# YiwenShaoStephen/mergeNet

Hardware: AMD Instinct MI355X
Metric: merged Mpixels/sec at 1024x2048 (speculative fast path; proven path: value_proven_path) (higher is better)
Workload: dtype f32

## Files before the change

mergenet_amd/csrc/mergenet_hip.hip:

```cpp
#include <hip/hip_runtime.h>
#include <hip/hip_ext.h>

#include <math.h>
#include <stdio.h>
#include <stdlib.h>
#include <string.h>
#include <time.h>

#include "../../include/mergenet_hip.h"
#include "mn_device.h"
#include "mn_kernels_score.h"
#include "mn_kernels_merge.h"
#include "mn_kernels_finish.h"
#include "mn_kernels_output.h"
#include "mn_kernels_prepare.h"
#include "mn_kernels_instances.h"
#include "mn_kernels_cc.h"
#include "mn_kernels_tail.h"
#include "mn_kernels_exact.h"
#include "mn_kernels_reforder.h"

#define MN_NSCALARS 16
#define MN_STAT_BYTES ((((sizeof(Counters) + 15) & ~(size_t)15)) + MN_NSCALARS * sizeof(int) + 4 * sizeof(double))

#define MN_MAX_SUBROUNDS 64

static thread_local int g_last_status = MN_OK;

#define MN_HIP(expr)                                                                      \
  do {                                                                                    \
    hipError_t _e = (expr);                                                               \
    if (_e != hipSuccess) {                                                               \
      fprintf(stderr, "mergenet_hip: %s failed: %s (%s:%d)\n", #expr, hipGetErrorString(_e), \
              __FILE__, __LINE__);                                                        \
      g_last_status = MN_ERR_NO_DEVICE;                                                   \
      return MN_ERR_NO_DEVICE;                                                            \
    }                                                                                     \
  } while (0)

template <typename T>
struct HostBuf {
  T* p;
  explicit HostBuf(size_t n) : p(static_cast<T*>(calloc(n ? n : 1, sizeof(T)))) {}
  ~HostBuf() { free(p); }
  HostBuf(const HostBuf&) = delete;
  bool ok() const { return p != nullptr; }
  operator T*() const { return p; }
};

struct ImageCall {
  const void *d_class, *d_adj;
  int dtype;
  int class_dim, offset_dim, W, H, num_classes;
  int *d_mask, *d_objcls, *d_part;
  hipStream_t stream;
  bool has_offsets;
  int offs[2 * MN_MAX_OFFSETS];
  mn_options opts;
};

struct Queued { int mode, rounds, finish_limit, N; long long R0; bool speculate, want_cert; };

struct mn_context {
  int device;
  int maxH, maxW, maxC, maxO;
  size_t N, Rmax, cap;
  size_t cap_full;
  int gen_ready;
  size_t gen_bytes;
  size_t cc_cap;
  int debug_flags;
  size_t bytes;
  unsigned char *ocls, *cls0, *lpvalid, *matched, *pruned;
  int *osize, *parent, *mate, *root, *label, *mapbuf;
  float* lpsum;
  i64* lp_acc;
  u64 *ball, *bsub;
  RecList LA, LB;
  int* touched_list;
  int* fin_lists;
  int fin_lds_ready, tail_lds_ready;
  int* wire_counts;
  int core_radius;
  int ext_events;
  int cores_used;
  int cc_clean;
  HashTab T;
  int* block_count;
  double* partial;
  Counters* cnt;
  int* scalars;
  unsigned* gmax;
  unsigned* touch;
  unsigned* h_touch;
  float* theta;
  int* progress;
  u64* bg_key;
  double* lp_out;
  Counters* h_cnt;
  int* h_scalars;
  double* h_lp;
  size_t cc_sum_lds, oc_lds;
  unsigned char* statblk;
  unsigned char* h_statblk;
  int *cc_tcount, *cc_lcount;
  unsigned* cc_bits;
  int* cc_roots;
  int cc_sign_blocks;
  unsigned* cc_negbits;
  size_t cc_cap_max;
  hipEvent_t ev[12];
  struct Pending {
    int active;
    int rc;
    Queued queued;
    ImageCall call;
    mn_stats stats;
  } pend;
  hipEvent_t ev_done;
  struct Replay {
    int state;
    int capturing;
    unsigned char key[256];
    size_t key_bytes;
    hipGraph_t gA, gB;
    hipGraphExec_t eA, eB;
    hipStream_t cap;
    Queued queued;
  } replay;
  hipStream_t side;
  hipEvent_t ev_fork;
  ImgParams last_params;
  int last_valid;
  struct XWork {
    XState X;
    size_t n_pix, n_rec, n_cls_floats, hcap, arena_cap, leaf_cap;
    void* block;
    size_t bytes;
    XCtl* h_ctl;
    int lds_ready;
    int prerun;
    ImgParams* d_P;
    XState* d_X;
    int batch_cap;
    int arena_extra;
    int table_permille;
    int max_blocks;
  } xw;
  struct RWork {
    RoState S;
    void* block;
    size_t bytes;
    int n_pix; long long n_rec; int n_cls; long long arena_cap, heap_cap;
    int arena_per_pixel, heap_per_record;
    long long* h_ctl;
    RoState* d_S;
    int batch_cap;
  } rw;
  int tie_ref;
  int tie_used;
  float *d_class, *d_same;
  int *d_mask, *d_objcls, *d_part;
};

#define MN_DEFAULT_CORE_RADIUS 6

static double g_host_us[4];
static long long g_host_n[2];
static inline double host_now_us() {
  timespec ts;
  clock_gettime(CLOCK_MONOTONIC, &ts);
  return (double)ts.tv_sec * 1e6 + (double)ts.tv_nsec * 1e-3;
}

struct HostLaunchTimer {
  double t0;
  HostLaunchTimer() : t0(host_now_us()) {}
  ~HostLaunchTimer() { g_host_us[0] += host_now_us() - t0; g_host_n[0]++; }
};

static size_t next_pow2(size_t x) {
  size_t p = 1;
  while (p < x) p <<= 1;
  return p;
}

template <typename T>
static hipError_t dev_alloc(mn_context* c, T** p, size_t n) {
  const size_t b = (n * sizeof(T) + 255) & ~(size_t)255;
  c->bytes += b;
  return hipMalloc(reinterpret_cast<void**>(p), b);
}

static void x_free(mn_context* c) {
  XState& X = c->xw.X;
  if (c->xw.block) (void)hipFree(c->xw.block);
  if (X.mlog) (void)hipFree(X.mlog);
  if (c->xw.h_ctl) (void)hipHostFree(c->xw.h_ctl);
  c->bytes -= c->xw.bytes;
  const mn_context::XWork keep = c->xw;
  memset(&c->xw, 0, sizeof(c->xw));
  c->xw.d_P = keep.d_P; c->xw.d_X = keep.d_X; c->xw.batch_cap = keep.batch_cap;
  c->xw.arena_extra = keep.arena_extra; c->xw.table_permille = keep.table_permille; c->xw.max_blocks = keep.max_blocks;
}

static void r_free(mn_context* c) {
  if (c->rw.block) (void)hipFree(c->rw.block);
  if (c->rw.h_ctl) (void)hipHostFree(c->rw.h_ctl);
  c->bytes -= c->rw.bytes;
  const int ap = c->rw.arena_per_pixel, hp = c->rw.heap_per_record, bc = c->rw.batch_cap;
  RoState* ds = c->rw.d_S;
  memset(&c->rw, 0, sizeof(c->rw));
  c->rw.arena_per_pixel = ap; c->rw.heap_per_record = hp; c->rw.d_S = ds; c->rw.batch_cap = bc;
}

static int x_ensure(mn_context* c, int N, int O, int C) {
  mn_context::XWork& w = c->xw;
  const size_t NL = (size_t)N * O;
  if (NL >= 0xFFFFFFF0ull) return MN_ERR_CAPACITY;
  size_t B = 256;
  const size_t max_blocks = w.max_blocks > 0 ? (size_t)w.max_blocks : (size_t)MN_X_MAXBLOCKS;
  while ((NL + B - 1) / B > max_blocks) B <<= 1;
  const size_t NB = (NL + B - 1) / B;
  const size_t leaf_cap = NB * B + 1024;
  if (w.arena_extra <= 0) {
    w.arena_extra = 8 * O + 8;
    if (const char* e = getenv("MN_X_ARENA_EXTRA")) { const int v = atoi(e); if (v > 0) w.arena_extra = v; }
    w.table_permille = 600;
    if (const char* e = getenv("MN_X_TABLE_PERMILLE")) { const int v = atoi(e); if (v >= 50 && v <= 950) w.table_permille = v; }
  }
  const size_t nbuckets = (size_t)((double)NL * 1000.0 / (4.0 * (double)w.table_permille)) + 64;
  if (nbuckets * 4 >= 0xFFFFFFF0ull) return MN_ERR_CAPACITY;
  const size_t arena_cap = (size_t)N * (size_t)w.arena_extra + 65536;
  if (arena_cap >= 0xFFFFFFF0ull) return MN_ERR_CAPACITY;
  const size_t ovf_cap = NL / 256 + 4096;
  if (w.n_pix < (size_t)N || w.n_rec < NL || w.n_cls_floats < (size_t)N * C || w.hcap < nbuckets ||
      w.arena_cap < arena_cap || w.leaf_cap < leaf_cap) {
    x_free(c);
    XState& X = w.X;
    {
      const size_t al = ((size_t)N * O > (1u << 20)) ? ((size_t)2 << 20) : 4096;
      size_t off = 0;
      auto take = [&](size_t bytes) { const size_t o = off; off += (bytes + al - 1) / al * al; return o; };
      const size_t o_hs = take(nbuckets * 4 * sizeof(XSlot)), o_rec = take(NL * sizeof(XRec)),
                   o_arena = take(arena_cap * sizeof(unsigned)), o_leaf = take(leaf_cap * sizeof(unsigned)),
                   o_lp = take(((size_t)N * C + 64) * sizeof(float)), o_obj = take((size_t)N * sizeof(XObj)),
                   o_acap = take((size_t)N * sizeof(int)), o_ostamp = take((size_t)N * 2 * sizeof(unsigned)),
                   o_ovf = take(ovf_cap * sizeof(unsigned)), o_l1g = take((size_t)MN_X_MAXBLOCKS * sizeof(u64)),
                   o_tstack = take((size_t)MN_X_TSTACK * sizeof(u64)), o_free = take((size_t)MN_X_FREE_CLASSES * sizeof(unsigned)),
                   o_ctl = take(sizeof(XCtl));
      MN_HIP(hipMalloc(&w.block, off));
      w.bytes = off;
      c->bytes += off;
      char* b = static_cast<char*>(w.block);
      X.hs = reinterpret_cast<XSlot*>(b + o_hs); X.rec = reinterpret_cast<XRec*>(b + o_rec);
      X.arena = reinterpret_cast<unsigned*>(b + o_arena); X.leaf = reinterpret_cast<unsigned*>(b + o_leaf);
      X.lp = reinterpret_cast<float*>(b + o_lp); X.obj = reinterpret_cast<XObj*>(b + o_obj);
      X.acap = reinterpret_cast<int*>(b + o_acap); X.ostamp = reinterpret_cast<unsigned*>(b + o_ostamp);
      X.overflow = reinterpret_cast<unsigned*>(b + o_ovf); X.l1g = reinterpret_cast<u64*>(b + o_l1g);
      X.tstack = reinterpret_cast<u64*>(b + o_tstack); X.ctl = reinterpret_cast<XCtl*>(b + o_ctl);
      X.freeheads = reinterpret_cast<unsigned*>(b + o_free);
    }
    MN_HIP(hipHostMalloc(reinterpret_cast<void**>(&w.h_ctl), sizeof(XCtl)));
    w.n_pix = N; w.n_rec = NL; w.n_cls_floats = (size_t)N * C; w.hcap = nbuckets; w.arena_cap = arena_cap;
    w.leaf_cap = leaf_cap;
    X.overflow_cap = (int)ovf_cap;
  }
  XState& X = w.X;
  X.nb = (unsigned)nbuckets;
  X.arena_cap = arena_cap;
  X.Blog = 0;
  while (((size_t)1 << X.Blog) < B) X.Blog++;
  X.NB = (int)NB;
  X.NBpad = (int)((NB + 63) / 64 * 64);
  X.NG = X.NBpad / 64;
  X.NL = (unsigned)NL;
  X.parent = c->parent;
  X.dbg = getenv("MN_X_FORCE_RELOCATE") ? 1 : 0;
  if (getenv("MN_X_MERGELOG") && !X.mlog) {
    if (hipMalloc(reinterpret_cast<void**>(&X.mlog), (size_t)N * 16) == hipSuccess) X.mlog_cap = N;
    else X.mlog = nullptr;
// ... 291 lines not shown
}

static int begin_call(mn_context* c, const ImageCall& call, bool entry_ok, mn_stats* stats, ImgParams* P) {
  int rc = check_args(c, call);
  if (rc == MN_OK && (!call.d_class || !call.d_adj || !dtype_ok(call.dtype, true) || !entry_ok)) rc = MN_ERR_ARGUMENT;
  if (stats) { memset(stats, 0, sizeof(*stats)); stats->status = rc; stats->total_logprob = NAN; }
  if (rc != MN_OK) { g_last_status = rc; return rc; }
  MN_HIP(hipSetDevice(c->device));
  fill_params(P, call);
  return MN_OK;
}

static long long count_records(const ImageCall& call) {
  long long r = 0;
  for (int k = 0; k < call.offset_dim; k++) {
    const long long hh = call.H - abs(call.offs[2 * k]), ww = call.W - abs(call.offs[2 * k + 1]);
    if (hh > 0 && ww > 0) r += hh * ww;
  }
  return r;
}

static inline unsigned grid_for(size_t n, unsigned block) { return (unsigned)((n + block - 1) / block); }

struct FillList {
  FillJobs j;
  size_t largest = 0;
  FillList() { j.count = 0; }
  void add(void* p, size_t bytes, unsigned char byte) {
    if (!bytes) return;
    j.ptr[j.count] = p;
    j.bytes[j.count] = bytes;
    j.pattern[j.count] = 0x01010101u * byte;
    j.count++;
    if (bytes > largest) largest = bytes;
  }
  bool full() const { return j.count == MN_FILL_JOBS; }
  void launch(hipStream_t st) {
    if (!j.count) return;
    unsigned blocks = grid_for(largest / 16 + 1, 256 * 4);
    if (blocks > 4096) blocks = 4096;
    if (blocks < 1) blocks = 1;
    hipLaunchKernelGGL(mn_fill_many, dim3(blocks), dim3(256), 0, st, j);
    j.count = 0;
    largest = 0;
  }
};

static ObjState obj_state(mn_context* c) {
  ObjState S;
  S.ocls = c->ocls; S.osize = c->osize; S.parent = c->parent; S.lpsum = c->lpsum;
  S.lpvalid = c->lpvalid;
  return S;
}

template <bool FIRST>
static void launch_edge_pass(mn_context* c, const ImgParams& P, hipStream_t st, u64* out, int s) {
  const int* progress = c->progress;
  const dim3 g(grid_for(P.N, 256)), b(256);
  const dim3 gx(8 * ((grid_for(P.N, 256) + 7) / 8));
  const unsigned char* cls0 = c->ocls;
  const unsigned char* matched = c->matched;
  const bool fast = P.omf > 0.0f && P.sdb == 0.0f && !(c->debug_flags & 1);
  if (fast && P.O == 10 && !P.clip)
    hipLaunchKernelGGL((mn_edge_pass_fast<10, FIRST, false>), gx, b, 0, st, P, cls0, matched, out,
                       progress, s);
  else if (fast && P.O == 10)
    hipLaunchKernelGGL((mn_edge_pass_fast<10, FIRST, true>), gx, b, 0, st, P, cls0, matched, out,
                       progress, s);
  else if (fast && P.O == 16 && !P.clip)
    hipLaunchKernelGGL((mn_edge_pass_fast<16, FIRST, false>), gx, b, 0, st, P, cls0, matched, out,
                       progress, s);
  else if (fast && P.O == 16)
    hipLaunchKernelGGL((mn_edge_pass_fast<16, FIRST, true>), gx, b, 0, st, P, cls0, matched, out,
                       progress, s);
  else
    hipLaunchKernelGGL(mn_edge_pass_generic<FIRST>, g, b, 0, st, P, obj_state(c), matched, out, progress, s);
}

static int run_phase_a(mn_context* c, const ImgParams& P, hipStream_t st, bool edge,
                       FillList* fills = nullptr, bool components = false) {
  const int N = P.N;
  FillList own;
  if (!fills) fills = &own;
  if (!components) {
    fills->add(c->lpvalid, N, 0);
    fills->add(c->matched, N, 0);
  }
  fills->launch(st);
  if (components) {
    if (!c->ext_events) MN_HIP(hipEventRecord(c->ev[0], st));
    return MN_OK;
  }
  hipLaunchKernelGGL(mn_init_objects, dim3(grid_for(N, 256)), dim3(256), 0, st, N, c->osize,
                     c->parent, c->mate);
  MN_HIP(hipEventRecord(c->ev[0], st));
  {
    const unsigned blocks = grid_for((size_t)(N >> 2) > 0 ? (size_t)(N >> 2) : 1, 256);
    hipLaunchKernelGGL(mn_class_pass, dim3(blocks), dim3(256), 0, st, P, c->ocls);
  }
  MN_HIP(hipEventRecord(c->ev[1], st));
  if (edge) {
    launch_edge_pass<true>(c, P, st, c->ball, 0);
  }
  MN_HIP(hipEventRecord(c->ev[2], st));
  MN_HIP(hipMemcpyAsync(c->cls0, c->ocls, N, hipMemcpyDeviceToDevice, st));
  MN_HIP(hipGetLastError());
  return MN_OK;
}

static int read_counters(mn_context* c, hipStream_t st) {
  MN_HIP(hipMemcpyAsync(c->h_cnt, c->cnt, sizeof(Counters), hipMemcpyDeviceToHost, st));
  MN_HIP(hipStreamSynchronize(st));
  return MN_OK;
}

static int build_list(mn_context* c, const ImgParams& P, hipStream_t st, size_t cap, RecList L,
                      const RecList* src, int Rsrc, int* Rout) {
  ObjState S = obj_state(c);
  HashTab T = c->T;
  T.mask = (unsigned)(cap - 1);
  FillList f;
  f.add(T.key, cap * sizeof(u64), 0xFF);
  f.add(T.S, cap * sizeof(i64), 0);
  f.add(T.touched, cap, 0);
  f.add(&c->cnt->n_records, sizeof(int), 0);
  f.add(c->ball, (size_t)P.N * sizeof(u64), 0);
  f.add(c->gmax, 64 * sizeof(unsigned), 0);
  f.launch(st);
  if (!src)
    hipLaunchKernelGGL(mn_build_from_pixels, dim3(grid_for(P.N, 256)), dim3(256), 0, st, P, S, T);
  else
    hipLaunchKernelGGL(mn_rebuild, dim3(grid_for(Rsrc, MN_REBUILD_ITEMS)), dim3(256), 0, st, S, *src,
                       Rsrc, (const unsigned char*)c->matched, T, L, c->ball, c->gmax, c->cnt,  0);
  if (cap <= (1u << 16))
    hipLaunchKernelGGL(mn_compact<1>, dim3(grid_for(cap, 256)), dim3(256), 0, st, P, S, T, L,
                       c->ball, c->gmax, c->cnt, (const int*)nullptr, (int*)nullptr);
  else
    hipLaunchKernelGGL(mn_compact<4>, dim3(grid_for(cap, MN_COMPACT_SLOTS)), dim3(256), 0, st, P, S, T, L,
                       c->ball, c->gmax, c->cnt, (const int*)nullptr, (int*)nullptr);
  MN_HIP(hipGetLastError());
  if (read_counters(c, st) != MN_OK) return MN_ERR_NO_DEVICE;
  *Rout = c->h_cnt->n_records;
  return MN_OK;
}

static size_t gsum_stride(int N) {
#ifdef MN_GSUM_SKEW
  return ((((size_t)N / 4 + 63) / 64) | 1) * 64;
#else
  return (size_t)N;
#endif
}

template <int PX, int DT, bool LG = false>
static void launch_sign(mn_context* c, const ImgParams& P, hipStream_t st, bool cls, bool lean_cls) {
  const int N = P.N, ngroups = (N + PX - 1) / PX;
  const dim3 g(grid_for(ngroups, MN_CC_SIGN_THREADS)), b(MN_CC_SIGN_THREADS);
  ClsOut CO;
  CO.ocls = lean_cls ? nullptr : c->ocls; CO.cls0 = c->cls0; CO.lpvalid = lean_cls ? nullptr : c->lpvalid;
  CO.gsum = reinterpret_cast<int*>(c->lpsum);
  CO.gstride = gsum_stride(P.N);
  const bool plain = (DT != MN_DTYPE_F32 || LG || !P.clip) && P.sdb == 0.0f;
#define MN_LAUNCH_SIGN(PLAINV, CLSV)                                                                    \
  do {                                                                                                \
    if (c->ext_events)                                                                                \
      hipExtLaunchKernelGGL((mn_cc_sign<PX, PLAINV, (CLSV) && PX >= 4, DT, LG>), g, b, 0, st, c->ev[0], c->ev[10], 0, \
                            P, c->cc_bits, c->cc_negbits, c->scalars + 6, c->partial, CO); \
    else                                                                                              \
      hipLaunchKernelGGL((mn_cc_sign<PX, PLAINV, (CLSV) && PX >= 4, DT, LG>), g, b, 0, st, P, c->cc_bits, c->cc_negbits, \
                         c->scalars + 6, c->partial, CO);                                             \
  } while (0)
  if (plain && cls) MN_LAUNCH_SIGN(true, true);
  else if (plain) MN_LAUNCH_SIGN(true, false);
  else if (cls) MN_LAUNCH_SIGN(false, true);
  else MN_LAUNCH_SIGN(false, false);
#undef MN_LAUNCH_SIGN
}

static int sweep_px(const mn_context* c, const ImgParams& P) {
  if (!((P.N & 3) == 0 && P.W >= 4)) return 1;
  if (P.dtype != MN_DTYPE_F32 && !(c->debug_flags & 256) && (P.N & 7) == 0 && (P.W & 7) == 0 &&
      ((reinterpret_cast<uintptr_t>(P.cls) | reinterpret_cast<uintptr_t>(P.same)) & 15) == 0)
    return 8;
  return 4;
}

template <bool LG>
static void launch_sweep_lg(mn_context* c, const ImgParams& P, hipStream_t st, int px, bool cls, bool lean_cls) {
#define MN_SWEEP_DT(PXV)                                                                         \
  do {                                                                                           \
    if (P.dtype == MN_DTYPE_F16) launch_sign<PXV, MN_DTYPE_F16, LG>(c, P, st, cls, lean_cls);    \
    else launch_sign<PXV, MN_DTYPE_BF16, LG>(c, P, st, cls, lean_cls);                           \
  } while (0)
  if (P.dtype == MN_DTYPE_F32) {
    if (px == 4) launch_sign<4, MN_DTYPE_F32, LG>(c, P, st, cls, lean_cls);
    else launch_sign<1, MN_DTYPE_F32, LG>(c, P, st, false, false);
  } else if (px == 8) MN_SWEEP_DT(8);
  else if (px == 4) MN_SWEEP_DT(4);
  else { cls = false; lean_cls = false; MN_SWEEP_DT(1); }
#undef MN_SWEEP_DT
}
static void launch_sweep(mn_context* c, const ImgParams& P, hipStream_t st, int px, bool cls, bool lean_cls) {
  if (P.logits) launch_sweep_lg<true>(c, P, st, px, cls, lean_cls);
  else launch_sweep_lg<false>(c, P, st, px, cls, lean_cls);
}

template <int PX>
static void launch_cc_hook(mn_context* c, const ImgParams& P, hipStream_t st, unsigned kmask,
                           const unsigned* hook_bits = nullptr, hipEvent_t hook_done = nullptr) {
  const int N = P.N, ngroups = (N + PX - 1) / PX;
  const dim3 gx(8 * ((grid_for(ngroups, 256) + 7) / 8));
  if (hook_done)
    hipExtLaunchKernelGGL(mn_cc_hook<PX>, gx, dim3(256), 0, st, nullptr, hook_done, 0, P,
                          hook_bits ? hook_bits : (const unsigned*)c->cc_bits, c->parent, kmask);
  else
    hipLaunchKernelGGL(mn_cc_hook<PX>, gx, dim3(256), 0, st, P, hook_bits ? hook_bits : (const unsigned*)c->cc_bits,
                       c->parent, kmask);
}

enum CcUse {
  CC_WAITED,
  CC_QUEUED_COMPACT,
  CC_QUEUED_TAIL,
  CC_CORES
};

static int run_components(mn_context* c, const ImgParams& P, hipStream_t& st, CcUse use) {
  const bool wait = use == CC_WAITED, with_ball = use == CC_WAITED;
  const bool with_compact = use == CC_WAITED || use == CC_QUEUED_COMPACT;
  const bool fork_before_sums = use == CC_QUEUED_TAIL, cores = use == CC_CORES;
  const int N = P.N;
  ObjState S = obj_state(c);
  const dim3 b(256);
  const bool four = P.W % 4 == 0;
  int kh = -1, kv = -1, dv = 0;
  for (int k = 0; k < P.O; k++) {
    if (kh < 0 && P.di[k] == 0 && P.dj[k] == 1) kh = k;
    if (kv < 0 && P.dj[k] == 0 && (P.di[k] == 1 || P.di[k] == -1)) { kv = k; dv = P.di[k]; }
  }
  const bool few_events = (c->debug_flags & 2) != 0;
  const bool lean = (c->debug_flags & 16) != 0;
  const dim3 tiles((P.W + 63) / 64, (P.H + MN_CC_TILE_ROWS - 1) / MN_CC_TILE_ROWS);
  const int px = sweep_px(c, P);
  const bool sweep4 = px >= 4;
  const size_t sign_blocks = grid_for((size_t)(N / px), MN_CC_SIGN_THREADS);
  c->cc_sign_blocks = (int)(sign_blocks * (MN_CC_SIGN_THREADS / 64));
  int* clsmin = c->root;
  int* clsmax = c->mapbuf;
  const bool fused_cls = sweep4;
  const bool lean_cls = fused_cls && !cores;
  launch_sweep(c, P, st, px, fused_cls, lean_cls);
  if (!few_events && !c->ext_events) MN_HIP(hipEventRecord(c->ev[10], st));
  const unsigned* lbits = c->cc_bits;
  unsigned kshort = 0u;
  if (cores) {
    if (!fused_cls) {
      const unsigned blocks = grid_for((size_t)(N >> 2) > 0 ? (size_t)(N >> 2) : 1, 256);
      hipLaunchKernelGGL(mn_class_pass, dim3(blocks), dim3(256), 0, st, P, c->cls0);
    }
    unsigned* bits2 = reinterpret_cast<unsigned*>(c->label);
    for (int k = 0; k < P.O; k++)
      if (c->core_radius < 0 || (abs(P.di[k]) <= c->core_radius && abs(P.dj[k]) <= c->core_radius)) kshort |= 1u << k;
    hipLaunchKernelGGL(mn_core_clean, dim3(grid_for(N, 256)), b, 0, st, P, (const unsigned*)c->cc_bits,
                       (const unsigned char*)c->cls0, c->pruned, kshort);
    hipLaunchKernelGGL(mn_core_bits, dim3(grid_for(N, 256)), b, 0, st, P, (const unsigned char*)c->pruned,
                       (const unsigned*)c->cc_bits, (const unsigned char*)c->cls0, bits2);
    lbits = bits2;
  }
  hipStream_t real = st;
  if (c->replay.capturing) {
    MN_HIP(hipStreamBeginCapture(c->replay.cap, hipStreamCaptureModeThreadLocal));
    st = c->replay.cap;
  }
  unsigned kmask = P.O >= 32 ? 0xFFFFFFFFu : ((1u << P.O) - 1u);
  const bool fork_ext = fork_before_sums && c->ext_events && !c->replay.capturing;
  bool fork_by_hook = false;
  hipLaunchKernelGGL(mn_cc_tiles, tiles, dim3(MN_CC_TILE_ROWS * 64), 0, st, P, lbits, c->parent, kh, kv, dv,
                     c->osize, c->lp_acc, clsmin, clsmax, c->matched);
  if (kh >= 0 || kv >= 0) {
    hipLaunchKernelGGL(mn_cc_borders, tiles, dim3(128), 0, st, P, lbits, c->parent, kh, kv, dv);
    if (kh >= 0) kmask &= ~(1u << kh);
    if (kv >= 0) kmask &= ~(1u << kv);
  }
  hipLaunchKernelGGL(mn_cc_flatten, dim3(grid_for((size_t)(N >> 2) > 0 ? (size_t)(N >> 2) : 1, 256)), b, 0, st, N, c->parent);
  fork_by_hook = fork_ext && kmask;
  if (kmask) {
    if (four) launch_cc_hook<4>(c, P, st, kmask, lbits, fork_by_hook ? c->ev_fork : nullptr);
    else launch_cc_hook<1>(c, P, st, kmask, lbits, fork_by_hook ? c->ev_fork : nullptr);
  }
  if (c->replay.capturing) {
    MN_HIP(hipStreamEndCapture(c->replay.cap, &c->replay.gA));
    MN_HIP(hipGraphInstantiate(&c->replay.eA, c->replay.gA, nullptr, nullptr, 0));
    MN_HIP(hipGraphLaunch(c->replay.eA, real));
    st = real;
  }
  HashTab T = c->T;
  T.mask = (unsigned)(c->cc_cap - 1);
  if (!few_events && !lean) MN_HIP(hipEventRecord(c->ev[7], st));
  if (fork_before_sums) {
    if (!fork_by_hook) MN_HIP(hipEventRecord(c->ev_fork, st));
    MN_HIP(hipStreamWaitEvent(c->side, c->ev_fork, 0));
    st = c->side;
    if (c->replay.capturing) {
      MN_HIP(hipStreamBeginCapture(c->replay.cap, hipStreamCaptureModeThreadLocal));
      st = c->replay.cap;
    }
  }
  if (!few_events && !lean) MN_HIP(hipEventRecord(c->ev[11], st));
  {
    const size_t lds = (size_t)MN_CC_SUM_SLOTS * (P.C + 1) * sizeof(u64);
    if (lds > c->cc_sum_lds) {
      MN_HIP(hipFuncSetAttribute(reinterpret_cast<const void*>(mn_cc_class_sums),
                                 hipFuncAttributeMaxDynamicSharedMemorySize, (int)lds));
      MN_HIP(hipFuncSetAttribute(reinterpret_cast<const void*>(mn_cc_sums),
                                 hipFuncAttributeMaxDynamicSharedMemorySize, (int)lds));
      c->cc_sum_lds = lds;
    }
    const unsigned blocks = grid_for((size_t)(N >> 2) > 0 ? (size_t)(N >> 2) : 1, MN_CC_SUM_THREADS);
    if (fused_cls)
      hipLaunchKernelGGL(mn_cc_sums, dim3((blocks + MN_CC_SUMS_ITERS - 1) / MN_CC_SUMS_ITERS), dim3(MN_CC_SUM_THREADS), lds, st, P, S,
                         (const unsigned char*)c->cls0, (const int*)reinterpret_cast<int*>(c->lpsum), gsum_stride(P.N),
                         c->lp_acc, clsmin, clsmax, cores ? (const unsigned char*)c->pruned : (const unsigned char*)nullptr);
    else
      hipLaunchKernelGGL(mn_cc_class_sums, dim3(blocks), dim3(MN_CC_SUM_THREADS), lds, st, P, S, c->cls0,
                         c->lp_acc, clsmin, clsmax);
  }
  if (!few_events && !lean) MN_HIP(hipEventRecord(c->ev[8], st));
  if (!cores)
  {
    if (sweep4)
      hipLaunchKernelGGL(mn_cc_cross<4>, dim3((unsigned)grid_for((size_t)N / 4, MN_CC_CROSS_THREADS)), dim3(MN_CC_CROSS_THREADS),
                         0, st, P, (const int*)c->parent, T, (const unsigned*)c->cc_negbits, c->scalars + 6, c->cc_tcount);
    else
      hipLaunchKernelGGL(mn_cc_cross<1>, dim3((unsigned)grid_for((size_t)N, MN_CC_CROSS_THREADS)), dim3(MN_CC_CROSS_THREADS),
                         0, st, P, (const int*)c->parent, T, (const unsigned*)c->cc_negbits, c->scalars + 6, c->cc_tcount);
  }
  if (!few_events && !lean) MN_HIP(hipEventRecord(c->ev[9], st));
  hipLaunchKernelGGL(mn_cc_finish, dim3(grid_for((size_t)(N >> 4) > 0 ? (size_t)(N >> 4) : 1, 256)), b, 0, st, P, S,
                     (const unsigned char*)c->matched, (const i64*)c->lp_acc,
                     (const int*)clsmin, (const int*)clsmax, c->mate, cores ? (int*)nullptr : c->cc_roots,
                     c->scalars + 8, c->scalars + 6, lean_cls ? (const unsigned char*)c->cls0 : (const unsigned char*)nullptr);
  if (cores) {
    const unsigned all = P.O >= 32 ? 0xFFFFFFFFu : ((1u << P.O) - 1u);
    if (kshort != all) {
      MN_HIP(hipMemsetAsync(c->matched, 0, (size_t)N, st));
      hipLaunchKernelGGL(mn_core_check, dim3(grid_for(N, 256)), b, 0, st, P, (const int*)c->parent, lbits, c->matched);
      hipLaunchKernelGGL(mn_core_dissolve, dim3(grid_for(N, 256)), b, 0, st, P, S,
                         (const unsigned char*)c->matched, c->scalars + 9);
    }
    hipLaunchKernelGGL(mn_count_cross_edges, dim3(grid_for(N, 256)), b, 0, st, P, (const int*)c->parent, c->touch);
  }
  if (with_compact)
    hipLaunchKernelGGL(mn_compact<4>, dim3(grid_for(c->cc_cap, MN_COMPACT_SLOTS)), dim3(256), 0, st, P, S,
                       T, c->LA, with_ball ? c->ball : (u64*)nullptr, c->gmax, c->cnt,
                       (const int*)c->cc_tcount, c->cc_lcount);
  MN_HIP(hipGetLastError());
  if (!wait) return 0;
  MN_HIP(hipMemcpyAsync(c->h_scalars, c->scalars, MN_NSCALARS * sizeof(int), hipMemcpyDeviceToHost, st));
  MN_HIP(hipMemcpyAsync(c->h_cnt, c->cnt, sizeof(Counters), hipMemcpyDeviceToHost, st));
  MN_HIP(hipStreamSynchronize(st));
  if (c->h_scalars[6] != 0 || c->h_scalars[7] != 0) {
    MN_HIP(hipMemsetAsync(c->cnt, 0, sizeof(Counters), st));
    return 1;
  }
  return 0;
}

static int exact_setup(mn_context* c, const ImgParams& P, hipStream_t st) {
  int rc = x_ensure(c, P.N, P.O, P.C);
  if (rc != MN_OK) return rc;
  mn_context::XWork& w = c->xw;
  XState& X = w.X;
  const size_t N = (size_t)P.N;
  MN_HIP(hipMemsetAsync(X.hs, 0xFF, (size_t)X.nb * 4 * sizeof(XSlot), st));
  MN_HIP(hipMemsetAsync(X.leaf, 0, (((size_t)X.NB << X.Blog) + 1024) * sizeof(unsigned), st));
  MN_HIP(hipMemsetAsync(X.ostamp, 0, (size_t)N * 2 * sizeof(unsigned), st));
  MN_HIP(hipMemsetAsync(X.freeheads, 0xFF, MN_X_FREE_CLASSES * sizeof(unsigned), st));
  memset(w.h_ctl, 0, sizeof(XCtl));
  w.h_ctl->ttrack = getenv("MN_X_NO_TIE_TRACKING") ? 0 : 1;
  w.h_ctl->bump = 0ull;
  MN_HIP(hipMemcpyAsync(X.ctl, w.h_ctl, sizeof(XCtl), hipMemcpyHostToDevice, st));
  hipLaunchKernelGGL(mn_x_init_objects, dim3(grid_for(N, 256)), dim3(256), 0, st, P, X, c->cls0);
  MN_HIP(hipEventRecord(c->ev[1], st));
  hipLaunchKernelGGL(mn_x_init_records, dim3(grid_for((size_t)X.NL, 256)), dim3(256), 0, st, P, X);
  MN_HIP(hipEventRecord(c->ev[2], st));
  MN_HIP(hipGetLastError());
  return MN_OK;
}

static int exact_loop(mn_context** cs, int n, const ImgParams* Ps, hipStream_t st, unsigned char* full) {
  mn_context::XWork& w0 = cs[0]->xw;
  if (w0.batch_cap < n) {
    if (w0.d_P) (void)hipFree(w0.d_P);
    if (w0.d_X) (void)hipFree(w0.d_X);
    w0.d_P = nullptr; w0.d_X = nullptr;
    MN_HIP(hipMalloc(reinterpret_cast<void**>(&w0.d_P), (size_t)n * sizeof(ImgParams)));
    MN_HIP(hipMalloc(reinterpret_cast<void**>(&w0.d_X), (size_t)n * sizeof(XState)));
    w0.batch_cap = n;
  }
  size_t lds = 0;
  long long max_total = 0;
  {
    HostBuf<XState> hx((size_t)n);
    if (!hx.ok()) return MN_ERR_INTERNAL;
    for (int i = 0; i < n; i++) {
      const XState& X = cs[i]->xw.X;
      hx[i] = X;
      const size_t l = MN_X_LDS_BYTES(X.NBpad);
      if (l > lds) lds = l;
      const long long mt = 8LL * (long long)X.NL + 65536;
      if (mt > max_total) max_total = mt;
    }
    hipError_t e1 = hipMemcpyAsync(w0.d_P, Ps, (size_t)n * sizeof(ImgParams), hipMemcpyHostToDevice, st);
    hipError_t e2 = hipMemcpyAsync(w0.d_X, hx, (size_t)n * sizeof(XState), hipMemcpyHostToDevice, st);
    hipError_t e3 = hipStreamSynchronize(st);
    MN_HIP(e1); MN_HIP(e2); MN_HIP(e3);
  }
  if (!w0.lds_ready) {
    MN_HIP(hipFuncSetAttribute(reinterpret_cast<const void*>(mn_x_run),
                               hipFuncAttributeMaxDynamicSharedMemorySize, 160 * 1024));
    w0.lds_ready = 1;
  }
  long long per_launch = 1LL << 24;
  if (const char* e = getenv("MN_X_BUDGET")) { const long long v = atoll(e); if (v > 0) per_launch = v; }
  const long long max_launches = 1 << 20;
  for (long long it = 0; it < max_launches; it++) {
    long long most = 0;
    bool any = false;
    for (int i = 0; i < n; i++) {
      mn_context::XWork& w = cs[i]->xw;
      if (it > 0 && w.h_ctl->status != MN_X_BUDGET) continue;
      any = true;
      if (w.h_ctl->steps > most) most = w.h_ctl->steps;
      hipLaunchKernelGGL(mn_x_build_l1, dim3(w.X.NB), dim3(64), 0, st, w.X);
    }
    if (!any) break;
    const long long left = max_total - most;
    if (left <= 0) {
      fprintf(stderr, "mergenet_hip: exact engine exceeded %lld steps\n", max_total);
      return MN_ERR_INTERNAL;
    }
    const long long budget = left < per_launch ? left : per_launch;
    hipLaunchKernelGGL(mn_x_run, dim3((unsigned)n), dim3(64), lds, st, (const ImgParams*)w0.d_P, (const XState*)w0.d_X, budget);
    MN_HIP(hipGetLastError());
    for (int i = 0; i < n; i++)
      MN_HIP(hipMemcpyAsync(cs[i]->xw.h_ctl, cs[i]->xw.X.ctl, sizeof(XCtl), hipMemcpyDeviceToHost, st));
    MN_HIP(hipStreamSynchronize(st));
    bool all_done = true;
    for (int i = 0; i < n; i++) {
      const int status = cs[i]->xw.h_ctl->status;
      if (status == MN_X_DONE) continue;
      all_done = false;
      if (status == MN_X_BUDGET) continue;
      if (status == MN_X_ARENA_FULL || status == MN_X_HASH_FULL) {
        if (getenv("MN_TRACE_EXACT"))
          fprintf(stderr, "exact engine: out of %s after %lld steps (image %d of the batch): workspace grows, run repeated\n",
                  status == MN_X_ARENA_FULL ? "adjacency arena" : "pair table", cs[i]->xw.h_ctl->steps, i);
        full[i] = (unsigned char)status;
        continue;
      }
      fprintf(stderr, "mergenet_hip: exact engine stopped with status %d after %lld steps\n", status, cs[i]->xw.h_ctl->steps);
      return MN_ERR_INTERNAL;
    }
    if (all_done) break;
  }
  for (int i = 0; i < n; i++)
    if (cs[i]->xw.h_ctl->status != MN_X_DONE && !full[i]) return MN_ERR_INTERNAL;
  return MN_OK;
}

static int exact_run(mn_context** cs, int n, const ImgParams* Ps, hipStream_t st) {
  HostBuf<mn_context*> sub((size_t)n); HostBuf<ImgParams> subP((size_t)n); HostBuf<unsigned char> full((size_t)n);
  int rc = (sub.ok() && subP.ok() && full.ok()) ? MN_OK : MN_ERR_INTERNAL, m = n;
  for (int i = 0; i < n && rc == MN_OK; i++) { sub[i] = cs[i]; subP[i] = Ps[i]; }
  for (int attempt = 0; rc == MN_OK && m > 0; attempt++) {
    if (attempt == 8) { rc = MN_ERR_CAPACITY; break; }
    for (int i = 0; i < m && rc == MN_OK; i++) rc = exact_setup(sub[i], subP[i], st);
    if (rc != MN_OK) break;
    memset(full, 0, (size_t)m);
    rc = exact_loop(sub, m, subP, st, full);
    if (rc != MN_OK) break;
    int k = 0;
    for (int i = 0; i < m; i++) {
      if (!full[i]) continue;
      mn_context::XWork& w = sub[i]->xw;
      if (full[i] == MN_X_ARENA_FULL) w.arena_extra *= 2;
      else if (w.table_permille > 100) w.table_permille = w.table_permille * 2 / 3;
      else { rc = MN_ERR_CAPACITY; break; }
// ... 561 lines not shown
                       A.cur, c->cc_lcount, c->label, c->fin_lists, c->cnt, max_steps, c->scalars, pl.finish_limit,
                       (const unsigned char*)c->cls0, (const int*)c->mate, (const int*)c->cc_roots, nbe,
                       (const double*)c->partial, c->lp_out, pl.want_cert ? 1 : 0, c->label, call.d_objcls);
  } else {
    if (A.mode != MN_MODE_EXACT && A.R > 0 && !call.opts.no_handover_refresh &&
        !(A.mode == MN_MODE_COMPONENTS && A.rounds == 0))
      hipLaunchKernelGGL(mn_rec_refresh, dim3(grid_for(A.R, 256)), dim3(256), 0, A.st, P, S, A.cur, A.R);
    if (A.R <= MN_FIN2_MAXR) {
      if (!c->fin_lds_ready) {
        MN_HIP(hipFuncSetAttribute(reinterpret_cast<const void*>(mn_finisher_lds),
                                   hipFuncAttributeMaxDynamicSharedMemorySize, MN_FIN2_MAXR * 12));
        c->fin_lds_ready = 1;
      }
      hipLaunchKernelGGL(mn_finisher_lds, dim3(1), dim3(MN_FIN2_THREADS), MN_FIN2_MAXR * 12, A.st, P, S, A.cur, A.R, c->label,
                         c->fin_lists, c->cnt, max_steps, pl.speculate ? (const int*)&c->cnt->n_records : (const int*)nullptr,
                         (const int*)(c->scalars + 6), pl.finish_limit,
                         (A.mode == MN_MODE_COMPONENTS && A.rounds == 0) ? c->cc_lcount : (int*)nullptr);
    } else {
      if (A.mode == MN_MODE_COMPONENTS || A.cores)
        MN_HIP(hipMemsetAsync(c->mapbuf, 0xFF, (size_t)P.N * sizeof(int), A.st));
      hipLaunchKernelGGL(mn_finisher, dim3(1), dim3(MN_FIN_THREADS), 0, A.st, P, S, A.cur, A.R, c->mapbuf,
                         c->touched_list, c->cnt, max_steps);
    }
  }
  if (!pl.lean) MN_HIP(hipEventRecord(c->ev[3], A.st));
  return MN_OK;
}

static int launch_output(mn_context* c, const ImgParams& P, const Plan& pl, const Attempt& A, const ImageCall& call) {
  const int N = P.N;
  const ObjState S = obj_state(c);
  const unsigned char* pruned = NULL;
  if (call.opts.variant == MN_VARIANT_PYSEGMENTER) {
    MN_HIP(hipMemsetAsync(c->bg_key, 0, sizeof(u64), A.st));
    hipLaunchKernelGGL(mn_prune_find_background, dim3(grid_for(N, 256)), dim3(256), 0, A.st, P, S, c->bg_key);
    hipLaunchKernelGGL(mn_prune_mark, dim3(grid_for(N, 256)), dim3(256), 0, A.st, P, S,
                       call.opts.prune_threshold, (const u64*)c->bg_key, c->pruned, c->cnt);
    pruned = c->pruned;
  }
  if (!pl.fused_tail) {
    const int nblk = (int)grid_for(N, MN_SCAN_ITEMS);
    hipLaunchKernelGGL(mn_rank_count, dim3(nblk), dim3(256), 0, A.st, N, S, pruned, c->block_count, c->scalars + 2);
    hipLaunchKernelGGL(mn_rank_scan, dim3(1), dim3(1024), 0, A.st, nblk, c->block_count, c->scalars + 1);
    hipLaunchKernelGGL(mn_rank_assign, dim3(nblk), dim3(256), 0, A.st, N, S, pruned,
                       (const int*)c->block_count, c->label, call.d_objcls);
  }
  {
    const bool need_root = pl.want_cert && !pl.fused_tail && !A.cc_certificate();
    int* root_out = need_root ? c->root : nullptr;
    const bool aligned = (N & 3) == 0 && ((reinterpret_cast<uintptr_t>(call.d_mask) | reinterpret_cast<uintptr_t>(call.d_objcls) |
                                           reinterpret_cast<uintptr_t>(call.d_part)) & 15) == 0;
    if (aligned)
      hipLaunchKernelGGL(mn_write_mask4, dim3(grid_for((size_t)N / 4, 256)), dim3(256), 0, A.st, N, (const int*)c->parent,
                         (const int*)c->label, (const int*)(c->scalars + 1), root_out, call.d_mask, call.d_part, call.d_objcls);
    else
      hipLaunchKernelGGL(mn_write_mask, dim3(grid_for(N, 256)), dim3(256), 0, A.st, N, (const int*)c->parent,
                         (const int*)c->label, (const int*)(c->scalars + 1), root_out, call.d_mask, call.d_part, call.d_objcls);
  }
  return MN_OK;
}

static int launch_certificate(mn_context* c, const ImgParams& P, const Plan& pl, const Attempt& A) {
  const int N = P.N, R = A.R;
  const ObjState S = obj_state(c);
  if (!pl.want_cert || pl.fused_tail) {
  } else if (A.cc_certificate()) {
    const int nbe = c->cc_sign_blocks;
    hipLaunchKernelGGL(mn_cc_certificate, dim3(1), dim3(MN_CC_CERT_THREADS), 0, A.st, P, S, (const unsigned char*)c->cls0,
                       (const int*)c->mate, (const int*)c->cc_roots, (const int*)(c->scalars + 8), nbe,
                       (const double*)c->partial, (const Counters*)c->cnt, c->lp_out, c->scalars);
  } else {
    const bool four = P.W % 4 == 0;
    const int vb = (int)grid_for(four ? (size_t)N / 4 : (size_t)N, four ? MN_VERIFY4_THREADS : 256);
    if (four)
      hipLaunchKernelGGL(mn_verify_edges4, dim3(vb), dim3(MN_VERIFY4_THREADS), 0, A.st, P, S,
                         (const unsigned char*)c->cls0, (const int*)c->root, c->partial, c->scalars);
    else
      hipLaunchKernelGGL(mn_verify_edges, dim3(vb), dim3(256), 0, A.st, P, S,
                         (const unsigned char*)c->cls0, (const int*)c->root, c->partial, c->scalars);
    hipLaunchKernelGGL(mn_verify_reduce, dim3(1), dim3(256), 0, A.st, vb, (const double*)c->partial, P.omf, c->lp_out);
    if (pl.xengine)
      hipLaunchKernelGGL(mn_x_verify_records, dim3(grid_for((size_t)c->xw.X.NL, 256)), dim3(256), 0, A.st, P,
                         c->xw.X, c->scalars);
  }
  if (pl.want_cert && !pl.fused_tail && R > 0)
    hipLaunchKernelGGL(mn_verify_records, dim3(grid_for(R, 256)), dim3(256), 0, A.st, P, S, A.cur, R,
                       c->scalars, pl.speculate ? (const int*)&c->cnt->n_records : (const int*)nullptr);
  if (!pl.lean) MN_HIP(hipEventRecord(c->ev[4], A.st));
  MN_HIP(hipGetLastError());
  return MN_OK;
}

static int close_attempt(mn_context* c, const ImageCall& call, const Plan& pl, Attempt& A, mn_stats* stats, bool defer) {
  hipStream_t st = A.st;
  const Queued q = {A.mode, A.rounds, pl.finish_limit, call.W * call.H, pl.R0, pl.speculate, pl.want_cert};
  MN_HIP(hipMemcpyAsync(c->h_statblk, c->statblk, MN_STAT_BYTES, hipMemcpyDeviceToHost, st));
  if (pl.fused_tail) {
    A.post.launch(st);
    c->cc_clean = 1;
  }
  if (c->replay.capturing) {
    MN_HIP(hipStreamEndCapture(c->replay.cap, &c->replay.gB));
    MN_HIP(hipGraphInstantiate(&c->replay.eB, c->replay.gB, nullptr, nullptr, 0));
    MN_HIP(hipGraphLaunch(c->replay.eB, c->side));
    st = c->side;
    c->replay.capturing = 0;
    c->replay.state = 2;
    c->replay.queued = q;
  }
  if (defer && pl.speculate) {
    MN_HIP(hipEventRecord(c->ev_done, st));
    c->pend.queued = q;
    return MN_PENDING;
  }
  MN_HIP(hipStreamSynchronize(st));
  return segment_read_back(c, &call.opts, q, stats);
}

static int segment_attempt(mn_context* c, const ImageCall& call, mn_stats* stats, int force_mode, bool speculate, bool defer = false) {
  ImgParams P;
  int rc = begin_call(c, call, call.d_mask && call.d_objcls, stats, &P);
  if (rc != MN_OK) return rc;
  static const int env_flags = getenv("MN_DEBUG_FLAGS_OR") ? atoi(getenv("MN_DEBUG_FLAGS_OR")) : 0;
  c->debug_flags = call.opts.debug_flags | env_flags;
  c->ext_events = !(call.opts.debug_flags & 2) && !(call.opts.debug_flags & 128);
  c->core_radius = call.opts.core_radius != 0 ? call.opts.core_radius : MN_DEFAULT_CORE_RADIUS;
  const Plan pl = make_plan(call, force_mode, speculate);
  c->tie_ref = pl.xengine ? call.opts.tie_order : MN_TIES_LOWEST_ID;
  c->tie_used = 0; c->cores_used = 0;
  if (!pl.xengine && (rc = ensure_fast(c)) != MN_OK) return rc;
  if (!pl.speculate && !pl.xengine && (rc = ensure_general(c)) != MN_OK) return rc;
  Attempt A = {call.stream, pl.mode, pl.mode == MN_MODE_ROUNDS && pl.cores_ok, c->LA, c->LB, 0, 0};
  build_clear_list(c, P, pl, A);
  if ((rc = run_first_phase(c, P, pl, A)) != MN_OK) return rc;
  if ((rc = run_round0(c, P, pl, A)) != MN_OK) return rc;
  if ((rc = run_rounds(c, P, pl, A)) != MN_OK) return rc;
  if ((rc = launch_finisher(c, P, pl, A, call)) != MN_OK) return rc;
  if ((rc = launch_output(c, P, pl, A, call)) != MN_OK) return rc;
  if ((rc = launch_certificate(c, P, pl, A)) != MN_OK) return rc;
  c->last_params = P; c->last_valid = 1;
  return close_attempt(c, call, pl, A, stats, defer);
}

static int replay_launch(mn_context* c, const ImageCall& call) {
  ImgParams P;
  const int rc = begin_call(c, call, true, nullptr, &P);
  if (rc != MN_OK) return rc;
  const hipStream_t st = call.stream;
  c->debug_flags = call.opts.debug_flags;
  c->ext_events = !(call.opts.debug_flags & 2) && !(call.opts.debug_flags & 128);
  c->cores_used = 0;
  const bool timed = !(call.opts.debug_flags & 2) && !c->ext_events;
  if (timed) MN_HIP(hipEventRecord(c->ev[0], st));
  launch_sweep(c, P, st, sweep_px(c, P), true, true);
  if (timed) MN_HIP(hipEventRecord(c->ev[10], st));
  MN_HIP(hipGraphLaunch(c->replay.eA, st));
  MN_HIP(hipEventRecord(c->ev_fork, st));
  MN_HIP(hipStreamWaitEvent(c->side, c->ev_fork, 0));
  MN_HIP(hipGraphLaunch(c->replay.eB, c->side));
  MN_HIP(hipEventRecord(c->ev_done, c->side));
  c->last_params = P; c->last_valid = 1;
  c->pend.queued = c->replay.queued;
  memset(&c->pend.stats, 0, sizeof(c->pend.stats));
  c->pend.active = 1;
  return MN_OK;
}

extern "C" int mn_segment_launch_t(mn_context* c, const void* d_class_pred, int class_dim,
                                   const void* d_adj_pred, int offset_dim, int dtype, int W, int H,
                                   int num_classes, const int* offset_list, int* d_mask,
                                   int* d_object_class, int* d_partition, const mn_options* opts,
                                   void* stream) {
  if (!c || c->pend.active || !dtype_ok(dtype, true)) { g_last_status = MN_ERR_ARGUMENT; return MN_ERR_ARGUMENT; }
  HostLaunchTimer host_timer;
  mn_context::Pending& q = c->pend;
  q.call = ImageCall{d_class_pred, d_adj_pred, dtype, class_dim, offset_dim, W, H, num_classes, d_mask, d_object_class, d_partition};
  image_call(&q.call, offset_list, opts, stream);
  const mn_options& o = q.call.opts;
  mn_context::Replay& rp = c->replay;
  const bool want_replay = (o.debug_flags & 32) && (o.debug_flags & 16) && offset_list &&
                           offset_dim > 0 && offset_dim <= MN_MAX_OFFSETS && W % 4 == 0;
  unsigned char key[256];
  size_t kb = 0;
  if (want_replay) {
    memset(key, 0, sizeof(key));
    const void* ptrs[6] = {d_class_pred, d_adj_pred, d_mask, d_object_class, d_partition, stream};
    const int dims[6] = {class_dim, offset_dim, W, H, num_classes, dtype};
    memcpy(key + kb, ptrs, sizeof(ptrs)); kb += sizeof(ptrs);
    memcpy(key + kb, dims, sizeof(dims)); kb += sizeof(dims);
    memcpy(key + kb, &o, sizeof(o)); kb += sizeof(o);
    const size_t ob = sizeof(int) * 2 * (size_t)offset_dim;
    if (kb + ob <= sizeof(key)) { memcpy(key + kb, q.call.offs, ob); kb += ob; } else kb = 0;
  }
  const bool same_key = want_replay && kb && rp.state >= 1 && rp.key_bytes == kb && memcmp(rp.key, key, kb) == 0;
  if (same_key && rp.state == 2 && c->cc_clean) return replay_launch(c, q.call);
  if (want_replay && kb && !same_key) drop_replay_graphs(rp);
  rp.capturing = (same_key && rp.state == 1 && c->cc_clean) ? 1 : 0;
  const int was_clean = c->cc_clean;
  const int rc = segment_attempt(c, q.call, &q.stats, 0, true, true);
  if (rp.capturing) {
    hipGraph_t open_graph = nullptr;
    if (hipStreamEndCapture(rp.cap, &open_graph) == hipSuccess && open_graph) (void)hipGraphDestroy(open_graph);
    (void)hipGetLastError();
    rp.capturing = 0;
    rp.state = 0;
  }
  if (want_replay && kb && rp.state == 0 && rc == MN_PENDING && was_clean && c->cc_clean &&
      o.variant == MN_VARIANT_CSEGMENT && (W * H) % 4 == 0) {
    memcpy(rp.key, key, kb);
    rp.key_bytes = kb;
    rp.state = 1;
  }
  if (rc == MN_PENDING) { q.active = 1; return MN_OK; }
  if (rc < 0 && rc != MN_ERR_NO_BACKGROUND) return rc;
  q.active = 2;
  q.rc = rc;
  return MN_OK;
}

extern "C" int mn_segment_launch(mn_context* c, const float* d_class_pred, int class_dim,
                                 const float* d_adj_pred, int offset_dim, int W, int H,
                                 int num_classes, const int* offset_list, int* d_mask,
                                 int* d_object_class, int* d_partition, const mn_options* opts,
                                 void* stream) {
  return mn_segment_launch_t(c, d_class_pred, class_dim, d_adj_pred, offset_dim, MN_DTYPE_F32, W, H, num_classes,
                             offset_list, d_mask, d_object_class, d_partition, opts, stream);
}

extern "C" int mn_segment_finish(mn_context* c, mn_stats* stats) {
  if (!c || !c->pend.active) { g_last_status = MN_ERR_ARGUMENT; return MN_ERR_ARGUMENT; }
  const double t_in = host_now_us();
  double t_synced = t_in;
  mn_context::Pending& q = c->pend;
  const mn_options& o = q.call.opts;
  int rc;
  const bool explicit_mode = o.mode == MN_MODE_EXACT || o.mode == MN_MODE_ROUNDS || o.mode == MN_MODE_COMPONENTS;
  const bool must_prove = o.require_proof > 0 || (o.require_proof == 0 && !explicit_mode);
  if (q.active == 2) {
    rc = q.rc;
  } else {
    MN_HIP(hipSetDevice(c->device));
    MN_HIP(hipEventSynchronize(c->ev_done));
    t_synced = host_now_us();
    memset(&q.stats, 0, sizeof(q.stats));
    rc = segment_read_back(c, &o, q.queued, &q.stats);
    if (rc == MN_RETRY_ROUNDS && must_prove)
      rc = segment_attempt(c, q.call, &q.stats, MN_MODE_EXACT, false);
    else if (rc == MN_RETRY_ROUNDS || rc == MN_RETRY_WAIT)
      rc = segment_attempt(c, q.call, &q.stats, rc == MN_RETRY_ROUNDS ? MN_MODE_ROUNDS : 0, false);
  }
  if (rc == MN_OK && must_prove && q.stats.proof == 0) {
    rc = segment_attempt(c, q.call, &q.stats, MN_MODE_EXACT, false);
    if (rc == MN_ERR_CAPACITY) rc = MN_ERR_UNPROVEN;
    if (rc == MN_ERR_UNPROVEN) { q.stats.status = rc; g_last_status = rc; }
  }
  if (rc == MN_OK && o.require_proof > 0 && q.stats.proof == MN_PROOF_SEQUENTIAL_TIES) {
    if (o.variant == MN_VARIANT_CSEGMENT) {
      ImageCall again = q.call;
      again.opts.tie_order = MN_TIES_REFERENCE;
      rc = segment_attempt(c, again, &q.stats, MN_MODE_EXACT, false);
      if (rc == MN_ERR_CAPACITY) rc = MN_ERR_UNPROVEN;
    } else {
      rc = MN_ERR_UNPROVEN;
    }
    if (rc == MN_ERR_UNPROVEN) { q.stats.status = rc; g_last_status = rc; }
  }
  if (stats) *stats = q.stats;
  q.active = 0;
  g_host_us[1] += t_synced - t_in; g_host_us[2] += host_now_us() - t_synced; g_host_n[1]++;
  return rc;
}

extern "C" int mn_segment_device_t(mn_context* c, const void* d_class_pred, int class_dim,
                                   const void* d_adj_pred, int offset_dim, int dtype, int W, int H,
                                   int num_classes, const int* offset_list, int* d_mask,
                                   int* d_object_class, int* d_partition, const mn_options* opts,
                                   void* stream, mn_stats* stats) {
  int rc = MN_ERR_ARGUMENT;
  if (!c || !c->pend.active)
    rc = mn_segment_launch_t(c, d_class_pred, class_dim, d_adj_pred, offset_dim, dtype, W, H, num_classes,
                             offset_list, d_mask, d_object_class, d_partition, opts, stream);
  if (rc != MN_OK) {
    if (stats) { memset(stats, 0, sizeof(*stats)); stats->status = rc; stats->total_logprob = NAN; }
    return rc;
  }
  return mn_segment_finish(c, stats);
}

extern "C" int mn_segment_device(mn_context* c, const float* d_class_pred, int class_dim,
                                 const float* d_adj_pred, int offset_dim, int W, int H,
                                 int num_classes, const int* offset_list, int* d_mask,
                                 int* d_object_class, int* d_partition, const mn_options* opts,
                                 void* stream, mn_stats* stats) {
  return mn_segment_device_t(c, d_class_pred, class_dim, d_adj_pred, offset_dim, MN_DTYPE_F32, W, H, num_classes,
                             offset_list, d_mask, d_object_class, d_partition, opts, stream, stats);
}

extern "C" int mn_segment_exact_batch_t(mn_context** ctxs, int count, const void* const* d_class_pred, int class_dim,
                                        const void* const* d_adj_pred, int offset_dim, int dtype, int W, int H,
                                        int num_classes, const int* offset_list, int* const* d_mask,
                                        int* const* d_object_class, int* const* d_partition, const mn_options* opts,
                                        void* stream, mn_stats* stats) {
  ImageCall shared = {nullptr, nullptr, dtype, class_dim, offset_dim, W, H, num_classes};
  image_call(&shared, offset_list, opts, stream);
  shared.opts.mode = MN_MODE_EXACT;
  const mn_options& o = shared.opts;
  if (!ctxs || count <= 0 || count > 4096 || !d_class_pred || !d_adj_pred || !d_mask || !d_object_class ||
// ... 58 lines not shown
    int n2 = 0;
    for (int i = 0; i < count; i++) {
      if (out[i].status != MN_OK || out[i].proof != MN_PROOF_SEQUENTIAL_TIES) continue;
      if (!ref_possible) {
        out[i].status = MN_ERR_UNPROVEN;
        if (rc == MN_OK) rc = MN_ERR_UNPROVEN;
        continue;
      }
      rc_ctx[n2] = ctxs[i]; rc_P[n2] = Ps[i]; rc_idx[n2] = i; n2++;
    }
    const int r2 = n2 > 0 ? redo_in_reference_order(rc_ctx, n2, rc_P, st, true) : MN_OK;
    if (r2 == MN_ERR_CAPACITY) {
      for (int j = 0; j < n2; j++) out[rc_idx[j]].status = MN_ERR_UNPROVEN;
      if (rc == MN_OK) rc = MN_ERR_UNPROVEN;
    } else if (r2 != MN_OK) {
      g_last_status = r2;
      return r2;
    }
    for (int j = 0; j < n2 && r2 == MN_OK; j++) {
      const int i = rc_idx[j];
      ctxs[i]->xw.prerun = 2;
      const int r = segment_attempt(ctxs[i], calls[i], &out[i], MN_MODE_EXACT, false);
      ctxs[i]->xw.prerun = 0;
      if (r != MN_OK && rc == MN_OK) rc = r;
    }
  }
  g_last_status = rc;
  return rc;
}

extern "C" int mn_segment_exact_batch(mn_context** ctxs, int count, const float* const* d_class_pred, int class_dim,
                                      const float* const* d_adj_pred, int offset_dim, int W, int H, int num_classes,
                                      const int* offset_list, int* const* d_mask, int* const* d_object_class,
                                      int* const* d_partition, const mn_options* opts, void* stream,
                                      mn_stats* stats) {
  return mn_segment_exact_batch_t(ctxs, count, reinterpret_cast<const void* const*>(d_class_pred), class_dim,
                                  reinterpret_cast<const void* const*>(d_adj_pred), offset_dim, MN_DTYPE_F32, W, H,
                                  num_classes, offset_list, d_mask, d_object_class, d_partition, opts, stream, stats);
}

extern "C" int mn_score_device_t(mn_context* c, const void* d_class_pred, int class_dim,
                                 const void* d_adj_pred, int offset_dim, int dtype, int W, int H,
                                 int num_classes, const int* offset_list, const mn_options* opts,
                                 void* stream, unsigned char* d_cls_out,
                                 unsigned long long* d_best_out, float* ms_class_pass,
                                 float* ms_edge_pass) {
  ImageCall call = {d_class_pred, d_adj_pred, dtype, class_dim, offset_dim, W, H, num_classes};
  image_call(&call, offset_list, opts, stream);
  ImgParams P;
  int rc = begin_call(c, call, true, nullptr, &P);
  if (rc != MN_OK) return rc;
  const hipStream_t st = call.stream;
  c->debug_flags = call.opts.debug_flags;
  if ((rc = ensure_fast(c)) != MN_OK || (rc = run_phase_a(c, P, st, true)) != MN_OK) return rc;
  if (d_cls_out) MN_HIP(hipMemcpyAsync(d_cls_out, c->ocls, P.N, hipMemcpyDeviceToDevice, st));
  if (d_best_out)
    MN_HIP(hipMemcpyAsync(d_best_out, c->ball, (size_t)P.N * sizeof(u64), hipMemcpyDeviceToDevice, st));
  MN_HIP(hipStreamSynchronize(st));
  float ms = 0;
  (void)hipEventElapsedTime(&ms, c->ev[0], c->ev[1]);
  if (ms_class_pass) *ms_class_pass = ms;
  (void)hipEventElapsedTime(&ms, c->ev[1], c->ev[2]);
  if (ms_edge_pass) *ms_edge_pass = ms;
  g_last_status = MN_OK;
  return MN_OK;
}

extern "C" int mn_score_device(mn_context* c, const float* d_class_pred, int class_dim,
                               const float* d_adj_pred, int offset_dim, int W, int H,
                               int num_classes, const int* offset_list, const mn_options* opts,
                               void* stream, unsigned char* d_cls_out,
                               unsigned long long* d_best_out, float* ms_class_pass,
                               float* ms_edge_pass) {
  return mn_score_device_t(c, d_class_pred, class_dim, d_adj_pred, offset_dim, MN_DTYPE_F32, W, H, num_classes,
                           offset_list, opts, stream, d_cls_out, d_best_out, ms_class_pass, ms_edge_pass);
}

extern "C" int mn_sweep_device_t(mn_context* c, const void* d_class_pred, int class_dim,
                                 const void* d_adj_pred, int offset_dim, int dtype, int W, int H, int num_classes,
                                 const int* offset_list, const mn_options* opts, void* stream,
                                 unsigned* d_bits_out, float* d_neg_out, unsigned char* d_cls_out,
                                 int* d_gsum_out, double* logsum_out, int* info_out) {
  ImageCall call = {d_class_pred, d_adj_pred, dtype, class_dim, offset_dim, W, H, num_classes};
  image_call(&call, offset_list, opts, stream);
  ImgParams P;
  const int rc = begin_call(c, call, d_bits_out && d_neg_out, nullptr, &P);
  if (rc != MN_OK) return rc;
  hipStream_t st = static_cast<hipStream_t>(stream);
  const int N = P.N;
  if (ensure_fast(c) != MN_OK) return MN_ERR_NO_DEVICE;
  c->debug_flags = call.opts.debug_flags | 2;
  c->ext_events = 0;
  c->cc_clean = 0;
  const int px = sweep_px(c, P);
  const bool four = px >= 4;
  const bool fused_cls = four;
  const size_t sign_blocks = grid_for((size_t)(N / px), MN_CC_SIGN_THREADS);
  const size_t sign_waves = sign_blocks * (MN_CC_SIGN_THREADS / 64);
  MN_HIP(hipMemsetAsync(c->scalars, 0, MN_NSCALARS * sizeof(int), st));
  launch_sweep(c, P, st, px, fused_cls, false);
  MN_HIP(hipMemsetD32Async(reinterpret_cast<hipDeviceptr_t>(d_neg_out), 0x7FC00000, (size_t)P.O * N, st));
  hipLaunchKernelGGL(mn_cc_export_neg, dim3((unsigned)grid_for((size_t)N, 256)), dim3(256), 0, st, P,
                     (const unsigned*)c->cc_negbits, d_neg_out);
  MN_HIP(hipMemcpyAsync(d_bits_out, c->cc_bits, (size_t)N * sizeof(unsigned), hipMemcpyDeviceToDevice, st));
  if (d_cls_out && fused_cls) MN_HIP(hipMemcpyAsync(d_cls_out, c->cls0, (size_t)N, hipMemcpyDeviceToDevice, st));
  if (d_gsum_out && fused_cls)
    MN_HIP(hipMemcpy2DAsync(d_gsum_out, (size_t)(N / 4) * sizeof(int), c->lpsum, gsum_stride(N) * sizeof(int),
                            (size_t)(N / 4) * sizeof(int), (size_t)P.C, hipMemcpyDeviceToDevice, st));
  HostBuf<double> hp(sign_waves * 2);
  if (!hp.ok()) return MN_ERR_INTERNAL;
  MN_HIP(hipMemcpyAsync(hp, c->partial, sign_waves * 2 * sizeof(double), hipMemcpyDeviceToHost, st));
  MN_HIP(hipMemcpyAsync(c->h_scalars, c->scalars, MN_NSCALARS * sizeof(int), hipMemcpyDeviceToHost, st));
  MN_HIP(hipStreamSynchronize(st));
  double t = 0.0;
  for (size_t b = 0; b < sign_waves; b++) t += hp[2 * b];
  if (logsum_out) *logsum_out = t;
  if (info_out) { info_out[0] = px; info_out[1] = fused_cls ? 1 : 0; info_out[2] = c->h_scalars[6]; }
  MN_HIP(hipGetLastError());
  g_last_status = MN_OK;
  return MN_OK;
}

extern "C" int mn_sweep_device(mn_context* c, const float* d_class_pred, int class_dim,
                               const float* d_adj_pred, int offset_dim, int W, int H, int num_classes,
                               const int* offset_list, const mn_options* opts, void* stream,
                               unsigned* d_bits_out, float* d_neg_out, unsigned char* d_cls_out,
                               int* d_gsum_out, double* logsum_out, int* info_out) {
  return mn_sweep_device_t(c, d_class_pred, class_dim, d_adj_pred, offset_dim, MN_DTYPE_F32, W, H, num_classes,
                           offset_list, opts, stream, d_bits_out, d_neg_out, d_cls_out, d_gsum_out, logsum_out, info_out);
}

extern "C" int mn_sweep_time_device_t(mn_context* c, const void* const* d_class_pred, const void* const* d_adj_pred,
                                      int dtype, int n_inputs, int class_dim, int offset_dim, int W, int H,
                                      int num_classes, const int* offset_list, const mn_options* opts, void* stream,
                                      int reps, float* us_per_launch) {
  const bool ok = d_class_pred && d_adj_pred && n_inputs >= 1 && reps >= 1 && us_per_launch;
  ImageCall call = {ok ? d_class_pred[0] : nullptr, ok ? d_adj_pred[0] : nullptr, dtype, class_dim, offset_dim, W, H, num_classes};
  image_call(&call, offset_list, opts, stream);
  ImgParams P;
  const int rc = begin_call(c, call, ok, nullptr, &P);
  if (rc != MN_OK) return rc;
  hipStream_t st = static_cast<hipStream_t>(stream);
  if (ensure_fast(c) != MN_OK) return MN_ERR_NO_DEVICE;
  c->debug_flags = call.opts.debug_flags | 2;
  c->ext_events = 0;
  c->cc_clean = 0;
  MN_HIP(hipMemsetAsync(c->scalars, 0, MN_NSCALARS * sizeof(int), st));
  for (int phase = 0; phase < 2; phase++) {
    const int n = phase == 0 ? (reps + 9) / 10 : reps;
    if (phase == 1) MN_HIP(hipEventRecord(c->ev[0], st));
    for (int i = 0; i < n; i++) {
      call.d_class = d_class_pred[i % n_inputs]; call.d_adj = d_adj_pred[i % n_inputs];
      fill_params(&P, call);
      launch_sweep(c, P, st, sweep_px(c, P), true, true);
    }
    if (phase == 1) MN_HIP(hipEventRecord(c->ev[1], st));
  }
  MN_HIP(hipStreamSynchronize(st));
  float ms = 0;
  MN_HIP(hipEventElapsedTime(&ms, c->ev[0], c->ev[1]));
  *us_per_launch = ms * 1e3f / (float)reps;
  MN_HIP(hipGetLastError());
  g_last_status = MN_OK;
  return MN_OK;
}

extern "C" int mn_sweep_time_device(mn_context* c, const float* const* d_class_pred, const float* const* d_adj_pred,
                                    int n_inputs, int class_dim, int offset_dim, int W, int H, int num_classes,
                                    const int* offset_list, const mn_options* opts, void* stream, int reps,
                                    float* us_per_launch) {
  return mn_sweep_time_device_t(c, reinterpret_cast<const void* const*>(d_class_pred),
                                reinterpret_cast<const void* const*>(d_adj_pred), MN_DTYPE_F32, n_inputs, class_dim,
                                offset_dim, W, H, num_classes, offset_list, opts, stream, reps, us_per_launch);
}

extern "C" int mn_exact_phase_a_device_t(mn_context* c, const void* d_class_pred, int class_dim,
                                         const void* d_adj_pred, int offset_dim, int dtype, int W, int H,
                                         int num_classes, const int* offset_list, const mn_options* opts,
                                         void* stream, unsigned char* d_cls_out, float* d_oml_out,
                                         float* d_prio_out) {
  ImageCall call = {d_class_pred, d_adj_pred, dtype, class_dim, offset_dim, W, H, num_classes};
  image_call(&call, offset_list, opts, stream);
  ImgParams P;
  int rc = begin_call(c, call, d_oml_out && d_prio_out, nullptr, &P);
  if (rc != MN_OK) return rc;
  hipStream_t st = static_cast<hipStream_t>(stream);
  if ((rc = exact_setup(c, P, st)) != MN_OK) { g_last_status = rc; return rc; }
  hipLaunchKernelGGL(mn_x_export_phase_a, dim3(grid_for((size_t)P.N * P.O, 256)), dim3(256), 0, st, P, c->xw.X,
                     d_oml_out, d_prio_out, d_cls_out);
  MN_HIP(hipGetLastError());
  MN_HIP(hipStreamSynchronize(st));
  g_last_status = MN_OK;
  return MN_OK;
}

extern "C" int mn_exact_phase_a_device(mn_context* c, const float* d_class_pred, int class_dim,
                                       const float* d_adj_pred, int offset_dim, int W, int H,
                                       int num_classes, const int* offset_list, const mn_options* opts,
                                       void* stream, unsigned char* d_cls_out, float* d_oml_out,
                                       float* d_prio_out) {
  return mn_exact_phase_a_device_t(c, d_class_pred, class_dim, d_adj_pred, offset_dim, MN_DTYPE_F32, W, H, num_classes,
                                   offset_list, opts, stream, d_cls_out, d_oml_out, d_prio_out);
}

static int ensure_staging(mn_context* c) {
  if (c->d_class) return MN_OK;
  MN_HIP(dev_alloc(c, &c->d_class, c->N * (size_t)c->maxC));
  MN_HIP(dev_alloc(c, &c->d_same, c->N * (size_t)c->maxO));
  MN_HIP(dev_alloc(c, &c->d_mask, c->N));
  MN_HIP(dev_alloc(c, &c->d_objcls, c->N));
  MN_HIP(dev_alloc(c, &c->d_part, c->N));
  return MN_OK;
}

extern "C" int mn_segment_host(mn_context* c, const float* class_pred, int class_dim,
                               const float* adj_pred, int offset_dim, int W, int H, int num_classes,
                               const int* offset_list, int* mask, int* object_class, int* partition,
                               const mn_options* opts, mn_stats* stats) {
  ImageCall call = {class_pred, adj_pred, MN_DTYPE_F32, class_dim, offset_dim, W, H, num_classes};
  image_call(&call, offset_list, opts, NULL);
  opts = &call.opts;
  int rc = check_args(c, call);
  if (rc == MN_OK && (!class_pred || !adj_pred || !mask || !object_class)) rc = MN_ERR_ARGUMENT;
  if (rc != MN_OK) { g_last_status = rc; if (stats) { memset(stats, 0, sizeof(*stats)); stats->status = rc; } return rc; }
  MN_HIP(hipSetDevice(c->device));
  rc = ensure_staging(c);
  if (rc != MN_OK) return rc;
  const size_t N = (size_t)W * H;
  MN_HIP(hipMemcpy(c->d_class, class_pred, N * num_classes * sizeof(float), hipMemcpyHostToDevice));
  MN_HIP(hipMemcpy(c->d_same, adj_pred, N * offset_dim * sizeof(float), hipMemcpyHostToDevice));
  rc = mn_segment_device(c, c->d_class, num_classes, c->d_same, offset_dim, W, H, num_classes,
                         offset_list, c->d_mask, c->d_objcls, c->d_part, opts, NULL, stats);
  if (rc != MN_OK && rc != MN_ERR_NO_BACKGROUND && rc != MN_ERR_UNPROVEN) return rc;
  MN_HIP(hipMemcpy(mask, c->d_mask, N * sizeof(int), hipMemcpyDeviceToHost));
  MN_HIP(hipMemcpy(object_class, c->d_objcls, N * sizeof(int), hipMemcpyDeviceToHost));
  if (partition) MN_HIP(hipMemcpy(partition, c->d_part, N * sizeof(int), hipMemcpyDeviceToHost));
  return rc;
}

extern "C" void c_run_segmentation(float* class_pred, int class_dim, float* adj_pred, int offset_dim,
                                   int img_width, int img_height, int num_classes, int* offset_list,
                                   int* output, int* object_class, float same_different_bias,
                                   float object_merge_factor, float merge_logprob_bias) {
  struct Cached { mn_context* c = NULL; ~Cached() { if (c) mn_destroy(c); } };
  static thread_local Cached holder;
  mn_context*& cached = holder.c;
  if (img_width <= 0 || img_height <= 0 || num_classes <= 0 || offset_dim <= 0) {
    g_last_status = MN_ERR_ARGUMENT;
    fprintf(stderr, "c_run_segmentation: %s\n", mn_status_string(MN_ERR_ARGUMENT));
    return;
  }
  if (cached && ((size_t)img_width * img_height > cached->N || num_classes > cached->maxC ||
                 offset_dim > cached->maxO)) {
    mn_destroy(cached);
    cached = NULL;
  }
  if (!cached) {
    int dev = 0;
    (void)hipGetDevice(&dev);
    cached = mn_create(dev, img_height, img_width, num_classes, offset_dim);
    if (!cached) {
      fprintf(stderr, "c_run_segmentation: %s\n", mn_status_string(g_last_status));
      return;
    }
  }
  mn_options o;
  mn_default_options(&o);
  o.same_different_bias = same_different_bias;
  o.object_merge_factor = object_merge_factor;
  o.merge_logprob_bias = merge_logprob_bias;
  const int rc = mn_segment_host(cached, class_pred, class_dim, adj_pred, offset_dim, img_width,
                                 img_height, num_classes, offset_list, output, object_class, NULL,
                                 &o, NULL);
  if (rc != MN_OK) fprintf(stderr, "c_run_segmentation: %s\n", mn_status_string(rc));
}


extern "C" int mn_prepare_device_t(mn_context* c, const void* d_in, int in_dtype, int channels, int in_height,
                                   int in_width, void* d_out, int out_dtype, int out_height, int out_width,
                                   int apply_sigmoid, int clip, void* stream) {
  if (!c || !d_in || !d_out || channels <= 0 || in_height <= 0 || in_width <= 0 || out_height <= 0 ||
      out_width <= 0 || out_height > 65535 || channels > 65535 || !dtype_ok(in_dtype, false) || !dtype_ok(out_dtype, false)) {
    g_last_status = MN_ERR_ARGUMENT;
    return MN_ERR_ARGUMENT;
  }
  MN_HIP(hipSetDevice(c->device));
  hipStream_t st = static_cast<hipStream_t>(stream);
  hipLaunchKernelGGL(mn_prepare_maps, dim3(grid_for(out_width, 256), out_height, channels), dim3(256),
                     0, st, d_in, in_dtype, channels, in_height, in_width, d_out, out_dtype, out_height, out_width,
                     apply_sigmoid, clip);
  MN_HIP(hipGetLastError());
  g_last_status = MN_OK;
  return MN_OK;
}

extern "C" int mn_prepare_device(mn_context* c, const float* d_in, int channels, int in_height,
                                 int in_width, float* d_out, int out_height, int out_width,
                                 int apply_sigmoid, int clip, void* stream) {
  return mn_prepare_device_t(c, d_in, MN_DTYPE_F32, channels, in_height, in_width, d_out, MN_DTYPE_F32, out_height,
                             out_width, apply_sigmoid, clip, stream);
}

extern "C" int mn_upsample_mask_device(mn_context* c, const int* d_mask, int in_height, int in_width,
                                       int* d_out, int out_height, int out_width, void* stream) {
  if (!c || !d_mask || !d_out || in_height <= 0 || in_width <= 0 || out_height <= 0 ||
      out_width <= 0 || out_height > 65535) {
    g_last_status = MN_ERR_ARGUMENT;
// ... 279 lines not shown
```

mergenet_amd/csrc/mn_kernels_cc.h:

```cpp
#pragma once

static_assert(MN_MAX_OFFSETS <= 32, "edge masks are 32-bit words: one bit per offset");

#include "mn_device.h"
#include "mn_kernels_merge.h"

#define MN_LP_FIX 16777216.0

__device__ __forceinline__ int mn_cc_find(int* __restrict__ parent, int x) {
  int p = parent[x];
  while (p != x) {
    const int g = parent[p];
    if (g != p) parent[x] = g;
    x = p;
    p = g;
  }
  return x;
}

struct __attribute__((packed, aligned(4))) mn_int4u { int x, y, z, w; };
__device__ __forceinline__ int4 mn_ld_int4_unaligned(const int* __restrict__ p) {
  const mn_int4u t = *reinterpret_cast<const mn_int4u*>(p);
  return make_int4(t.x, t.y, t.z, t.w);
}

#define MN_CC_SIGN_THREADS 256
#define MN_CC_SIGN_G 5
#define MN_CC_EDGE_PIXBITS 26

typedef float mn_f4v __attribute__((ext_vector_type(4)));
typedef unsigned mn_u4v __attribute__((ext_vector_type(4)));
__device__ __forceinline__ float4 mn_ld_stream4(const float* p) {
#ifdef MN_NT_LOADS
  const mn_f4v t = __builtin_nontemporal_load(reinterpret_cast<const mn_f4v*>(p));
  return make_float4(t.x, t.y, t.z, t.w);
#else
  return *reinterpret_cast<const float4*>(p);
#endif
}
typedef unsigned mn_u2v __attribute__((ext_vector_type(2)));
template <int DT, bool LG = false>
__device__ __forceinline__ float4 mn_ld_stream4_t(const void* base, size_t i) {
  if constexpr (LG) {
    return mn_sigmoid4(mn_ld_stream4_t<DT, false>(base, i));
  } else if constexpr (DT == MN_DTYPE_F32) {
    return mn_ld_stream4(static_cast<const float*>(base) + i);
  } else {
    const mn_u2v* q = reinterpret_cast<const mn_u2v*>(static_cast<const mn_u16*>(base) + i);
#ifdef MN_NT_LOADS
    const mn_u2v t = __builtin_nontemporal_load(q);
#else
    const mn_u2v t = *q;
#endif
    const float2 a = mn_widen2<DT>(t.x), b = mn_widen2<DT>(t.y);
    return make_float4(a.x, a.y, b.x, b.y);
  }
}
template <int DT, bool LG = false>
__device__ __forceinline__ void mn_ld_stream8_t(const void* base, size_t i, float* v) {
  static_assert(DT != MN_DTYPE_F32, "8 values per load: 16-bit maps only");
  const mn_u4v* q = reinterpret_cast<const mn_u4v*>(static_cast<const mn_u16*>(base) + i);
#ifdef MN_NT_LOADS
  const mn_u4v t = __builtin_nontemporal_load(q);
#else
  const mn_u4v t = *q;
#endif
  const float2 a = mn_widen2<DT>(t.x), b = mn_widen2<DT>(t.y), c = mn_widen2<DT>(t.z), d = mn_widen2<DT>(t.w);
  v[0] = a.x; v[1] = a.y; v[2] = b.x; v[3] = b.y; v[4] = c.x; v[5] = c.y; v[6] = d.x; v[7] = d.y;
  if constexpr (LG) {
#pragma unroll
    for (int j = 0; j < 8; j++) v[j] = mn_sigmoid(v[j]);
  }
}
template <int DT, bool LG = false>
__device__ __forceinline__ float mn_ld_stream1_t(const void* base, size_t i) {
  if constexpr (LG) return mn_sigmoid(mn_ld_stream1_t<DT, false>(base, i));
  else if constexpr (DT == MN_DTYPE_F32) return static_cast<const float*>(base)[i];
  else return mn_widen<DT>(static_cast<const mn_u16*>(base)[i]);
}
__device__ __forceinline__ void mn_st_stream(int* p, int v) {
#ifdef MN_NT_STORES
  __builtin_nontemporal_store(v, p);
#else
  *p = v;
#endif
}
__device__ __forceinline__ void mn_st_stream(uint4* p, uint4 v) {
#ifdef MN_NT_STORES
  mn_u4v t; t.x = v.x; t.y = v.y; t.z = v.z; t.w = v.w;
  __builtin_nontemporal_store(t, reinterpret_cast<mn_u4v*>(p));
#else
  *p = v;
#endif
}

template <bool PLAIN, int DT = MN_DTYPE_F32, bool LG = false>
__device__ __forceinline__ float mn_cc_value(const ImgParams& P, float v) {
  return PLAIN ? ((DT == MN_DTYPE_F32 && !LG) ? v : mn_clip(v)) : mn_same_value(P, v);
}

struct ClsOut {
  unsigned char* ocls; unsigned char* cls0; unsigned char* lpvalid; int* gsum; size_t gstride;
};

__device__ __forceinline__ int mn_cc_argmax_logf(const ImgParams& P, int p) {
  float best = 0.0f;
  int b = 0;
  for (int c = 0; c < P.C; c++) {
    const float l = logf(mn_ld_class(P, c, p));
    if (c == 0 || l > best) { best = l; b = c; }
  }
  return b;
}

template <int DT, bool LG = false>
__device__ __forceinline__ int mn_cc_argmax_logf_t(const ImgParams& P, int p) {
  float best = 0.0f;
  int b = 0;
  for (int c = 0; c < P.C; c++) {
    float v = mn_ld_stream1_t<DT, LG>(P.cls, (size_t)c * P.N + p);
    if (P.clip) v = mn_clip(v);
    const float l = logf(v);
    if (c == 0 || l > best) { best = l; b = c; }
  }
  return b;
}

template <int DT, bool LG = false>
__device__ __forceinline__ void mn_cc_class_part(const ImgParams& P, const ClsOut& CO, int i) {
  float4 best, prev = make_float4(-1.0f, -1.0f, -1.0f, -1.0f);
  int b0 = 0, b1 = 0, b2 = 0, b3 = 0;
  float4 nxt = mn_ld_stream4_t<DT, LG>(P.cls, 4 * (size_t)i);
  for (int c = 0; c < P.C; c++) {
    float4 v = nxt;
    if (c + 1 < P.C)
      nxt = mn_ld_stream4_t<DT, LG>(P.cls, (size_t)(c + 1) * P.N + 4 * (size_t)i);
    if (P.clip) { v.x = mn_clip(v.x); v.y = mn_clip(v.y); v.z = mn_clip(v.z); v.w = mn_clip(v.w); }
    if (c == 0) {
      best = v;
    } else {
      if (v.x > best.x) { prev.x = best.x; best.x = v.x; b0 = c; }
      if (v.y > best.y) { prev.y = best.y; best.y = v.y; b1 = c; }
      if (v.z > best.z) { prev.z = best.z; best.z = v.z; b2 = c; }
      if (v.w > best.w) { prev.w = best.w; best.w = v.w; b3 = c; }
    }
    mn_st_stream(&CO.gsum[(size_t)c * CO.gstride + i], __float2int_rn(logf((v.x * v.y) * (v.z * v.w)) * 16777216.0f));
  }
  const float near = 1.0f - 3.814697265625e-06f;
  if (prev.x >= best.x * near) b0 = mn_cc_argmax_logf_t<DT, LG>(P, 4 * i);
  if (prev.y >= best.y * near) b1 = mn_cc_argmax_logf_t<DT, LG>(P, 4 * i + 1);
  if (prev.z >= best.z * near) b2 = mn_cc_argmax_logf_t<DT, LG>(P, 4 * i + 2);
  if (prev.w >= best.w * near) b3 = mn_cc_argmax_logf_t<DT, LG>(P, 4 * i + 3);
  uchar4 o;
  o.x = (unsigned char)b0; o.y = (unsigned char)b1; o.z = (unsigned char)b2; o.w = (unsigned char)b3;
  if (CO.ocls) *reinterpret_cast<uchar4*>(CO.ocls + 4 * (size_t)i) = o;
  *reinterpret_cast<uchar4*>(CO.cls0 + 4 * (size_t)i) = o;
  if (CO.lpvalid) *reinterpret_cast<uchar4*>(CO.lpvalid + 4 * (size_t)i) = make_uchar4(0, 0, 0, 0);
}

template <int DT, bool LG = false>
__device__ __forceinline__ void mn_cc_class_part8(const ImgParams& P, const ClsOut& CO, int i) {
  float best[8], prev[8];
  int b[8];
#pragma unroll
  for (int j = 0; j < 8; j++) { best[j] = 0.0f; prev[j] = -1.0f; b[j] = 0; }
  float nxt[8];
  mn_ld_stream8_t<DT, LG>(P.cls, 8 * (size_t)i, nxt);
  for (int c = 0; c < P.C; c++) {
    float v[8];
#pragma unroll
    for (int j = 0; j < 8; j++) v[j] = mn_clip(nxt[j]);
    if (c + 1 < P.C) mn_ld_stream8_t<DT, LG>(P.cls, (size_t)(c + 1) * P.N + 8 * (size_t)i, nxt);
#pragma unroll
    for (int j = 0; j < 8; j++) {
      if (c == 0) best[j] = v[j];
      else if (v[j] > best[j]) { prev[j] = best[j]; best[j] = v[j]; b[j] = c; }
    }
    int2 g;
    g.x = __float2int_rn(logf((v[0] * v[1]) * (v[2] * v[3])) * 16777216.0f);
    g.y = __float2int_rn(logf((v[4] * v[5]) * (v[6] * v[7])) * 16777216.0f);
    *reinterpret_cast<int2*>(&CO.gsum[(size_t)c * CO.gstride + 2 * (size_t)i]) = g;
  }
  const float near = 1.0f - 3.814697265625e-06f;
#pragma unroll
  for (int j = 0; j < 8; j++)
    if (prev[j] >= best[j] * near) b[j] = mn_cc_argmax_logf_t<DT, LG>(P, 8 * i + j);
  uint2 o;
  o.x = (unsigned)b[0] | ((unsigned)b[1] << 8) | ((unsigned)b[2] << 16) | ((unsigned)b[3] << 24);
  o.y = (unsigned)b[4] | ((unsigned)b[5] << 8) | ((unsigned)b[6] << 16) | ((unsigned)b[7] << 24);
  if (CO.ocls) *reinterpret_cast<uint2*>(CO.ocls + 8 * (size_t)i) = o;
  *reinterpret_cast<uint2*>(CO.cls0 + 8 * (size_t)i) = o;
  if (CO.lpvalid) *reinterpret_cast<uint2*>(CO.lpvalid + 8 * (size_t)i) = make_uint2(0u, 0u);
}

template <int PX, bool PLAIN, bool CLS, int DT = MN_DTYPE_F32, bool LG = false>
__global__ __launch_bounds__(MN_CC_SIGN_THREADS) void mn_cc_sign(
    ImgParams P, unsigned* __restrict__ bits, unsigned* __restrict__ negbits, int* __restrict__ violations,
    double* __restrict__ partial, ClsOut CO) {
  const int lane = threadIdx.x & 63, wave = threadIdx.x >> 6;
  const int ngroups = (P.N + PX - 1) / PX;
  const int i = blockIdx.x * MN_CC_SIGN_THREADS + threadIdx.x;
  const bool live = i < ngroups;
  const int p0 = live ? PX * i : 0;
  const int r = p0 / P.W, c0 = p0 - r * P.W;
  if constexpr (CLS) {
    if (live) {
      if constexpr (PX == 8) mn_cc_class_part8<DT, LG>(P, CO, i);
      else mn_cc_class_part<DT, LG>(P, CO, i);
    }
  }
  float f = 1.0f;
  double t_sum = 0.0;
  unsigned m[PX], ng[PX];
#pragma unroll
  for (int j = 0; j < PX; j++) { m[j] = 0u; ng[j] = 0u; }
  unsigned inmask[PX];
#pragma unroll
  for (int j = 0; j < PX; j++) inmask[j] = 0u;
  constexpr int G = MN_CC_SIGN_G;
  const bool colsafe = live && c0 + P.djmin >= 0 && c0 + PX - 1 + P.djmax < P.W;
  const bool fast = __all(colsafe);
  const bool straddle = PX == 4 && live && c0 + PX - 1 >= P.W;
  unsigned rowmask = 0u;
  for (int k0 = 0; k0 < P.O; k0 += G) {
    float v[G][PX];
    int first[G];
    int rin[G];
#pragma unroll
    for (int g = 0; g < G; g++) {
      const int k = k0 + g;
      first[g] = INT_MIN;
      rin[g] = 0;
#pragma unroll
      for (int j = 0; j < PX; j++) v[g][j] = 1.0f;
      if (live && k < P.O) {
        const int rr = r + P.di[k];
        const bool in1 = rr >= 0 && rr < P.H, in2 = straddle && rr + 1 >= 0 && rr + 1 < P.H;
        if (in1 || in2) {
          first[g] = c0 + P.dj[k];
          rin[g] = (in1 ? 1 : 0) | (in2 ? 2 : 0);
          if (in1) rowmask |= 1u << k;
          if constexpr (PX == 8) {
            mn_ld_stream8_t<DT, LG>(P.same, (size_t)k * P.N + p0, v[g]);
          } else if (PX == 4) {
            const float4 t = mn_ld_stream4_t<DT, LG>(P.same, (size_t)k * P.N + p0);
            v[g][0] = t.x; v[g][1 % PX] = t.y; v[g][2 % PX] = t.z; v[g][3 % PX] = t.w;
          } else {
            v[g][0] = mn_ld_stream1_t<DT, LG>(P.same, (size_t)k * P.N + p0);
          }
        }
      }
    }
    if (fast) {
#pragma unroll
      for (int g = 0; g < G; g++) {
        const unsigned bit = (k0 + g < P.O) ? (1u << ((k0 + g) & 31)) : 0u;
#pragma unroll
        for (int j = 0; j < PX; j++) {
          const float x = ((PLAIN && DT == MN_DTYPE_F32 && !LG) || first[g] != INT_MIN) ? mn_cc_value<PLAIN, DT, LG>(P, v[g][j]) : 1.0f;
          m[j] |= (x >= P.sep_hi) ? bit : 0u;
          ng[j] |= (x <= P.sep_lo) ? bit : 0u;
          f *= fmaxf(x, 1.0f - x);
        }
      }
    } else {
#pragma unroll
      for (int g = 0; g < G; g++) {
        const unsigned bit = (k0 + g < P.O) ? (1u << ((k0 + g) & 31)) : 0u;
#pragma unroll
        for (int j = 0; j < PX; j++) {
          const bool second = straddle && c0 + j >= P.W;
          const bool inb = ((rin[g] >> (second ? 1 : 0)) & 1) &&
                           (unsigned)(first[g] + j - (second ? P.W : 0)) < (unsigned)P.W;
          const float x = inb ? mn_cc_value<PLAIN, DT, LG>(P, v[g][j]) : 1.0f;
          inmask[j] |= inb ? bit : 0u;
          m[j] |= (x >= P.sep_hi) ? bit : 0u;
          ng[j] |= (x <= P.sep_lo) ? bit : 0u;
          f *= fmaxf(x, 1.0f - x);
        }
      }
    }
    constexpr int FOLD = PX == 8 ? 1 : 3;
    if (((k0 / G) & FOLD) == FOLD || k0 + G >= P.O) {
      t_sum += (double)logf(f);
      f = 1.0f;
    }
  }
  int bad = 0;
#pragma unroll
  for (int j = 0; j < PX; j++) {
    const unsigned in = fast ? rowmask : inmask[j];
    m[j] &= in;
    ng[j] &= in;
    bad += __popc(in & ~(m[j] | ng[j]));
  }
  if (live) {
    if (PX == 8) {
      mn_st_stream(reinterpret_cast<uint4*>(bits + p0), make_uint4(m[0], m[1 % PX], m[2 % PX], m[3 % PX]));
      mn_st_stream(reinterpret_cast<uint4*>(bits + p0) + 1, make_uint4(m[4 % PX], m[5 % PX], m[6 % PX], m[7 % PX]));
      mn_st_stream(reinterpret_cast<uint4*>(negbits + p0), make_uint4(ng[0], ng[1 % PX], ng[2 % PX], ng[3 % PX]));
      mn_st_stream(reinterpret_cast<uint4*>(negbits + p0) + 1, make_uint4(ng[4 % PX], ng[5 % PX], ng[6 % PX], ng[7 % PX]));
    } else if (PX == 4) {
      mn_st_stream(reinterpret_cast<uint4*>(bits + p0), make_uint4(m[0], m[1 % PX], m[2 % PX], m[3 % PX]));
      mn_st_stream(reinterpret_cast<uint4*>(negbits + p0), make_uint4(ng[0], ng[1 % PX], ng[2 % PX], ng[3 % PX]));
    } else {
      bits[p0] = m[0];
      negbits[p0] = ng[0];
    }
  }
  for (int off = 32; off > 0; off >>= 1) {
    bad += __shfl_xor(bad, off);
    t_sum += __shfl_xor(t_sum, off);
  }
  if (lane == 0) {
    if (bad) atomicAdd(violations, bad);
    const size_t waveg = (size_t)blockIdx.x * (MN_CC_SIGN_THREADS / 64) + wave;
    partial[waveg * 2] = t_sum;
    partial[waveg * 2 + 1] = 0.0;
  }
}

__global__ __launch_bounds__(256) void mn_cc_export_neg(ImgParams P, const unsigned* __restrict__ negbits,
                                                        float* __restrict__ out) {
  const int p = blockIdx.x * 256 + threadIdx.x;
  if (p >= P.N) return;
  unsigned left = negbits[p];
  while (left) {
    const int k = __ffs((int)left) - 1;
    left &= left - 1u;
    const float x = mn_same_value(P, mn_ld_same(P, k, p));
    out[(size_t)k * P.N + p] = logf(x) - mn_log1m(x);
  }
}

#ifndef MN_CC_TILE_ROWS
#define MN_CC_TILE_ROWS 16
#endif
__global__ __launch_bounds__(MN_CC_TILE_ROWS * 64) void mn_cc_tiles(ImgParams P, const unsigned* __restrict__ bits,
                                                    int* __restrict__ parent, int kh, int kv, int dv,
                                                    int* __restrict__ osize, i64* __restrict__ lp_acc,
                                                    int* __restrict__ clsmin, int* __restrict__ clsmax,
                                                    unsigned char* __restrict__ cand) {
  __shared__ int lab[MN_CC_TILE_ROWS * 64];
  const int t = threadIdx.x, lane = t & 63, i = t >> 6;
  const int r = (int)blockIdx.y * MN_CC_TILE_ROWS + i, c = (int)blockIdx.x * 64 + lane;
  const bool in = r < P.H && c < P.W;
  const int p = in ? r * P.W + c : 0;
  const unsigned b = in ? bits[p] : 0u;
  const bool link = kh >= 0 && ((b >> kh) & 1u) && lane < 63;
  const int ni = i + dv;
  const bool vlink = kv >= 0 && ((b >> kv) & 1u) && ni >= 0 && ni < MN_CC_TILE_ROWS;
  const u64 m = __ballot(link);
  const u64 below = lane ? (~m & ((1ull << lane) - 1ull)) : 0ull;
  const int start = below ? (64 - __clzll((long long)below)) : 0;
  lab[t] = i * 64 + start;
  __syncthreads();
  int a = 0, bb = 0;
  bool want = false;
  if (vlink) {
    a = mn_cc_find(lab, t);
    bb = mn_cc_find(lab, ni * 64 + lane);
    want = a != bb;
  }
  u64 todo = __ballot(want);
  const u64 key = mn_key(a, bb);
  while (todo) {
    const int first = __ffsll((long long)todo) - 1;
    const u64 k0v = ((u64)(unsigned)__shfl((int)(key >> 32), first) << 32) |
                    (u64)(unsigned)__shfl((int)(key & 0xFFFFFFFFull), first);
    const bool mine = want && key == k0v;
    if (lane == first) {
      while (a != bb) {
        if (a < bb) { const int x = a; a = bb; bb = x; }
        const int old = atomicMin(&lab[a], bb);
        if (old == a) break;
        a = mn_cc_find(lab, old);
        bb = mn_cc_find(lab, bb);
      }
    }
    todo &= ~__ballot(mine);
  }
  __syncthreads();
  if (!in) return;
  int x = t;
  while (lab[x] != x) x = lab[x];
  parent[p] = ((int)blockIdx.y * MN_CC_TILE_ROWS + (x >> 6)) * P.W + (int)blockIdx.x * 64 + (x & 63);
  cand[p] = (x == t) ? 1 : 0;
  if (x == t) {
    osize[p] = 0;
    for (int c = 0; c < P.C; c++) lp_acc[(size_t)c * P.N + p] = 0;
    clsmin[p] = 255;
    clsmax[p] = 0;
  }
}

__device__ __forceinline__ void mn_cc_wave_union(int* __restrict__ parent, bool want, int a, int b) {
  const int lane = threadIdx.x & 63;
  u64 todo = __ballot(want);
  const u64 key = mn_key(a, b);
  while (todo) {
    const int first = __ffsll((long long)todo) - 1;
    const u64 k0v = ((u64)(unsigned)__shfl((int)(key >> 32), first) << 32) |
                    (u64)(unsigned)__shfl((int)(key & 0xFFFFFFFFull), first);
    const bool mine = want && key == k0v;
    if (lane == first) {
      while (a != b) {
        if (a < b) { const int t = a; a = b; b = t; }
        const int old = atomicMin(&parent[a], b);
        if (old == a) break;
        a = mn_cc_find(parent, old);
        b = mn_cc_find(parent, b);
      }
    }
    todo &= ~__ballot(mine);
  }
}

__global__ __launch_bounds__(128) void mn_cc_borders(ImgParams P, const unsigned* __restrict__ bits,
                                                     int* __restrict__ parent, int kh, int kv, int dv) {
  const int lane = threadIdx.x & 63, wave = threadIdx.x >> 6;
  const int r0 = (int)blockIdx.y * MN_CC_TILE_ROWS, c0 = (int)blockIdx.x * 64;
  int p = -1, q = -1;
  if (wave == 0) {
    const int r = r0 + lane, c = c0 + 63;
    if (kh >= 0 && lane < MN_CC_TILE_ROWS && r < P.H && c + 1 < P.W) {
      p = r * P.W + c;
      if ((bits[p] >> kh) & 1u) q = p + 1;
    }
  } else {
    const int r = dv > 0 ? r0 + MN_CC_TILE_ROWS - 1 : r0, c = c0 + lane;
    if (kv >= 0 && r < P.H && r + dv >= 0 && r + dv < P.H && c < P.W) {
      p = r * P.W + c;
      if ((bits[p] >> kv) & 1u) q = p + dv * P.W;
    }
  }
  int a = 0, b = 0;
  bool want = false;
  if (q >= 0) {
    a = mn_cc_find(parent, p);
    b = mn_cc_find(parent, q);
    want = a != b;
  }
  mn_cc_wave_union(parent, want, a, b);
}

__global__ __launch_bounds__(256) void mn_cc_flatten(int N, int* __restrict__ parent) {
  const int i = blockIdx.x * blockDim.x + threadIdx.x;
  const int n4 = N >> 2;
  if (i < n4) {
    int4 r = *reinterpret_cast<const int4*>(parent + 4 * (size_t)i);
    int4 o = r;
    int x = r.x; while (parent[x] != x) x = parent[x]; o.x = x;
    if (r.y == r.x) o.y = o.x; else { x = r.y; while (parent[x] != x) x = parent[x]; o.y = x; }
    if (r.z == r.x) o.z = o.x; else { x = r.z; while (parent[x] != x) x = parent[x]; o.z = x; }
    if (r.w == r.x) o.w = o.x; else { x = r.w; while (parent[x] != x) x = parent[x]; o.w = x; }
    if (o.x != r.x || o.y != r.y || o.z != r.z || o.w != r.w)
      *reinterpret_cast<int4*>(parent + 4 * (size_t)i) = o;
  }
  if (i < N - (n4 << 2)) {
    const int p = (n4 << 2) + i;
// ... 239 lines not shown
  const int i = blockIdx.x * MN_CC_SUM_THREADS + threadIdx.x;
  if (i < n4) {
    int4 r = *reinterpret_cast<const int4*>(S.parent + 4 * (size_t)i);
    r.x = mn_cc_root_ro(S.parent, r.x);
    r.y = r.y == r.x ? r.x : mn_cc_root_ro(S.parent, r.y);
    r.z = r.z == r.x ? r.x : mn_cc_root_ro(S.parent, r.z);
    r.w = r.w == r.x ? r.x : mn_cc_root_ro(S.parent, r.w);
    *reinterpret_cast<int4*>(S.parent + 4 * (size_t)i) = r;
    *reinterpret_cast<uchar4*>(S.lpvalid + 4 * (size_t)i) = make_uchar4(0, 0, 0, 0);
    const bool same = r.x == r.y && r.x == r.z && r.x == r.w;
    const int s0 = mn_lds_root_slot(s_root, r.x);
    const int s1 = same ? s0 : mn_lds_root_slot(s_root, r.y);
    const int s2 = same ? s0 : mn_lds_root_slot(s_root, r.z);
    const int s3 = same ? s0 : mn_lds_root_slot(s_root, r.w);
    float4 best, prev = make_float4(-1.0f, -1.0f, -1.0f, -1.0f);
    int b0 = 0, b1 = 0, b2 = 0, b3 = 0;
    float4 ring[MN_CC_SUM_AHEAD];
#pragma unroll
    for (int a = 0; a < MN_CC_SUM_AHEAD; a++)
      ring[a] = a < P.C ? mn_ld_class4(P, a, 4 * i)
                        : make_float4(0.5f, 0.5f, 0.5f, 0.5f);
    for (int c0 = 0; c0 < P.C; c0 += MN_CC_SUM_AHEAD) {
#pragma unroll
    for (int a = 0; a < MN_CC_SUM_AHEAD; a++) {
      const int c = c0 + a;
      if (c >= P.C) break;
      float4 v = ring[a];
      if (c + MN_CC_SUM_AHEAD < P.C)
        ring[a] = mn_ld_class4(P, (c + MN_CC_SUM_AHEAD), 4 * i);
      if (P.clip) { v.x = mn_clip(v.x); v.y = mn_clip(v.y); v.z = mn_clip(v.z); v.w = mn_clip(v.w); }
      if (c == 0) {
        best = v;
      } else {
        if (v.x > best.x) { prev.x = best.x; best.x = v.x; b0 = c; }
        if (v.y > best.y) { prev.y = best.y; best.y = v.y; b1 = c; }
        if (v.z > best.z) { prev.z = best.z; best.z = v.z; b2 = c; }
        if (v.w > best.w) { prev.w = best.w; best.w = v.w; b3 = c; }
      }
      if (same) {
        const float l = logf((v.x * v.y) * (v.z * v.w));
        mn_cc_add(P, S, s_root, s_val, lp_acc, r.x, c, s0, (i64)__float2int_rn(l * (float)MN_LP_FIX));
      } else {
        mn_cc_add(P, S, s_root, s_val, lp_acc, r.x, c, s0, (i64)__float2int_rn(logf(v.x) * (float)MN_LP_FIX));
        mn_cc_add(P, S, s_root, s_val, lp_acc, r.y, c, s1, (i64)__float2int_rn(logf(v.y) * (float)MN_LP_FIX));
        mn_cc_add(P, S, s_root, s_val, lp_acc, r.z, c, s2, (i64)__float2int_rn(logf(v.z) * (float)MN_LP_FIX));
        mn_cc_add(P, S, s_root, s_val, lp_acc, r.w, c, s3, (i64)__float2int_rn(logf(v.w) * (float)MN_LP_FIX));
      }
    }
    }
    const float near = 1.0f - 3.814697265625e-06f;
    if (prev.x >= best.x * near) b0 = mn_cc_argmax_logf(P, 4 * i);
    if (prev.y >= best.y * near) b1 = mn_cc_argmax_logf(P, 4 * i + 1);
    if (prev.z >= best.z * near) b2 = mn_cc_argmax_logf(P, 4 * i + 2);
    if (prev.w >= best.w * near) b3 = mn_cc_argmax_logf(P, 4 * i + 3);
    if (same) {
      mn_cc_add(P, S, s_root, s_val, lp_acc, r.x, P.C, s0, 4);
    } else {
      mn_cc_add(P, S, s_root, s_val, lp_acc, r.x, P.C, s0, 1);
      mn_cc_add(P, S, s_root, s_val, lp_acc, r.y, P.C, s1, 1);
      mn_cc_add(P, S, s_root, s_val, lp_acc, r.z, P.C, s2, 1);
      mn_cc_add(P, S, s_root, s_val, lp_acc, r.w, P.C, s3, 1);
    }
    uchar4 o;
    o.x = (unsigned char)b0; o.y = (unsigned char)b1; o.z = (unsigned char)b2; o.w = (unsigned char)b3;
    *reinterpret_cast<uchar4*>(S.ocls + 4 * (size_t)i) = o;
    *reinterpret_cast<uchar4*>(cls0 + 4 * (size_t)i) = o;
    if (same) {
      mn_cc_cls(s_min, s_max, clsmin, clsmax, r.x, s0, min(min(b0, b1), min(b2, b3)), max(max(b0, b1), max(b2, b3)));
    } else {
      mn_cc_cls(s_min, s_max, clsmin, clsmax, r.x, s0, b0, b0);
      mn_cc_cls(s_min, s_max, clsmin, clsmax, r.y, s1, b1, b1);
      mn_cc_cls(s_min, s_max, clsmin, clsmax, r.z, s2, b2, b2);
      mn_cc_cls(s_min, s_max, clsmin, clsmax, r.w, s3, b3, b3);
    }
  }
  const int tail0 = n4 << 2;
  if (i < P.N - tail0) {
    const int p = tail0 + i;
    const int root = mn_cc_root_ro(S.parent, p);
    S.parent[p] = root;
    S.lpvalid[p] = 0;
    float best = 0.0f;
    int b = 0;
    for (int c = 0; c < P.C; c++) {
      const float l = logf(mn_ld_class(P, c, p));
      if (c == 0 || l > best) { best = l; b = c; }
      mn_cc_add(P, S, s_root, s_val, lp_acc, root, c, -1, (i64)__float2int_rn(l * (float)MN_LP_FIX));
    }
    mn_cc_add(P, S, s_root, s_val, lp_acc, root, P.C, -1, 1);
    S.ocls[p] = (unsigned char)b;
    cls0[p] = (unsigned char)b;
    mn_cc_cls(s_min, s_max, clsmin, clsmax, root, -1, b, b);
  }
  __syncthreads();
  if (threadIdx.x < MN_CC_SUM_SLOTS && s_root[threadIdx.x] >= 0) {
    atomicMin(&clsmin[s_root[threadIdx.x]], s_min[threadIdx.x]);
    atomicMax(&clsmax[s_root[threadIdx.x]], s_max[threadIdx.x]);
  }
  for (int j = threadIdx.x; j < nval; j += MN_CC_SUM_THREADS) {
    const u64 v = s_val[j];
    if (v == 0) continue;
    const int slot = j / (P.C + 1), c = j - slot * (P.C + 1);
    mn_cc_add(P, S, s_root, s_val, lp_acc, s_root[slot], c, -1, (i64)v);
  }
}



__device__ __forceinline__ i64 mn_row16_sum(i64 x) {
  int lo = (int)(x & 0xFFFFFFFFll), hi = (int)(x >> 32);
#define MN_DPP_STEP(CTRL)                                                                   \
  {                                                                                         \
    const int lo2 = __builtin_amdgcn_update_dpp(0, lo, CTRL, 0xF, 0xF, false);              \
    const int hi2 = __builtin_amdgcn_update_dpp(0, hi, CTRL, 0xF, 0xF, false);              \
    const i64 y = ((i64)hi << 32 | (i64)(unsigned)lo) + ((i64)hi2 << 32 | (i64)(unsigned)lo2); \
    lo = (int)(y & 0xFFFFFFFFll); hi = (int)(y >> 32);                                      \
  }
  MN_DPP_STEP(0xB1)
  MN_DPP_STEP(0x4E)
  MN_DPP_STEP(0x141)
  MN_DPP_STEP(0x140)
#undef MN_DPP_STEP
  return (i64)hi << 32 | (i64)(unsigned)lo;
}

__device__ __forceinline__ i64 mn_rows4_sum(i64 rs) {
  const int lo = (int)(rs & 0xFFFFFFFFll), hi = (int)(rs >> 32);
  i64 t = 0;
#pragma unroll
  for (int k = 0; k < 4; k++)
    t += (i64)__builtin_amdgcn_readlane(hi, 16 * k) << 32 | (i64)(unsigned)__builtin_amdgcn_readlane(lo, 16 * k);
  return t;
}

__device__ __forceinline__ int mn_row16_min(int x) {
  x = min(x, __builtin_amdgcn_update_dpp(x, x, 0xB1, 0xF, 0xF, false));
  x = min(x, __builtin_amdgcn_update_dpp(x, x, 0x4E, 0xF, 0xF, false));
  x = min(x, __builtin_amdgcn_update_dpp(x, x, 0x141, 0xF, 0xF, false));
  x = min(x, __builtin_amdgcn_update_dpp(x, x, 0x140, 0xF, 0xF, false));
  return x;
}

__device__ __forceinline__ void mn_cc_sums_pixelwise(const ImgParams& P, const ObjState& S, int* s_root,
                                                  u64* s_val, i64* __restrict__ lp_acc, int4 r, int c,
                                                  int s0, int s1, int s2, int s3, float4 v) {
  const float vx = P.clip ? mn_clip(v.x) : v.x, vy = P.clip ? mn_clip(v.y) : v.y;
  const float vz = P.clip ? mn_clip(v.z) : v.z, vw = P.clip ? mn_clip(v.w) : v.w;
  mn_cc_add(P, S, s_root, s_val, lp_acc, r.x, c, s0, (i64)__float2int_rn(logf(vx) * (float)MN_LP_FIX));
  mn_cc_add(P, S, s_root, s_val, lp_acc, r.y, c, s1, (i64)__float2int_rn(logf(vy) * (float)MN_LP_FIX));
  mn_cc_add(P, S, s_root, s_val, lp_acc, r.z, c, s2, (i64)__float2int_rn(logf(vz) * (float)MN_LP_FIX));
  mn_cc_add(P, S, s_root, s_val, lp_acc, r.w, c, s3, (i64)__float2int_rn(logf(vw) * (float)MN_LP_FIX));
}

__global__ __launch_bounds__(MN_CC_SUM_THREADS) void mn_cc_sums(
    ImgParams P, ObjState S, const unsigned char* __restrict__ cls0, const int* __restrict__ gsum,
    size_t gstride, i64* __restrict__ lp_acc, int* __restrict__ clsmin, int* __restrict__ clsmax,
    const unsigned char* __restrict__ clean) {
  extern __shared__ __attribute__((aligned(16))) unsigned char cc_smem[];
  u64* s_val = reinterpret_cast<u64*>(cc_smem);
  __shared__ int s_root[MN_CC_SUM_SLOTS];
  __shared__ int s_min[MN_CC_SUM_SLOTS];
  __shared__ int s_max[MN_CC_SUM_SLOTS];
  __shared__ int s_q[MN_CC_SUM_THREADS * MN_CC_SUMS_ITERS];
  __shared__ int s_qn;
  const int nval = MN_CC_SUM_SLOTS * (P.C + 1);
  for (int i = threadIdx.x; i < nval; i += MN_CC_SUM_THREADS) s_val[i] = 0;
  if (threadIdx.x == 0) s_qn = 0;
  if (threadIdx.x < MN_CC_SUM_SLOTS) { s_root[threadIdx.x] = -1; s_min[threadIdx.x] = 255; s_max[threadIdx.x] = 0; }
  __syncthreads();
  const int n4 = P.N >> 2;
  for (int base = blockIdx.x * MN_CC_SUM_THREADS; base < n4; base += gridDim.x * MN_CC_SUM_THREADS) {
  const int i = base + (int)threadIdx.x;
  if (i < n4) {
    constexpr int G = MN_CC_SUMS_G;
    int4 r = *reinterpret_cast<const int4*>(S.parent + 4 * (size_t)i);
    const int4 r_in = r;
    const uchar4 b = *reinterpret_cast<const uchar4*>(cls0 + 4 * (size_t)i);
    int g[G];
#pragma unroll
    for (int a = 0; a < G; a++) g[a] = a < P.C ? gsum[(size_t)a * gstride + i] : 0;
    r.x = mn_cc_root_ro(S.parent, r.x);
    r.y = r.y == r.x ? r.x : mn_cc_root_ro(S.parent, r.y);
    r.z = r.z == r.x ? r.x : mn_cc_root_ro(S.parent, r.z);
    r.w = r.w == r.x ? r.x : mn_cc_root_ro(S.parent, r.w);
    if (r.x != r_in.x || r.y != r_in.y || r.z != r_in.z || r.w != r_in.w)
      *reinterpret_cast<int4*>(S.parent + 4 * (size_t)i) = r;
    const bool same = r.x == r.y && r.x == r.z && r.x == r.w;
    const int s0 = mn_lds_root_slot(s_root, r.x);
    const bool uni = __all(same && r.x == __shfl(r.x, 0) && i - (int)(threadIdx.x & 63) + 63 < n4);
    if (same) {
      const int lane = threadIdx.x & 63;
      for (int c0 = 0; c0 < P.C; c0 += G) {
        if (c0 > 0) {
#pragma unroll
          for (int a = 0; a < G; a++) g[a] = c0 + a < P.C ? gsum[(size_t)(c0 + a) * gstride + i] : 0;
        }
#pragma unroll
        for (int a = 0; a < G; a++) {
          if (c0 + a >= P.C) break;
          if (uni) {
#if MN_CC_SUMS_WAVE
            const i64 ws = mn_rows4_sum(mn_row16_sum((i64)g[a]));
            if (lane == 0) mn_cc_add(P, S, s_root, s_val, lp_acc, r.x, c0 + a, s0, ws);
#else
            const i64 rs = mn_row16_sum((i64)g[a]);
            if ((lane & 15) == 0) mn_cc_add(P, S, s_root, s_val, lp_acc, r.x, c0 + a, s0, rs);
#endif
          } else {
            mn_cc_add(P, S, s_root, s_val, lp_acc, r.x, c0 + a, s0, (i64)g[a]);
          }
        }
      }
      const int lo1 = min(min((int)b.x, (int)b.y), min((int)b.z, (int)b.w));
      const int hi1 = max(max((int)b.x, (int)b.y), max((int)b.z, (int)b.w));
      if (uni) {
#if MN_CC_SUMS_WAVE
        int lo = mn_row16_min(lo1), hi = -mn_row16_min(-hi1);
        lo = min(min(__builtin_amdgcn_readlane(lo, 0), __builtin_amdgcn_readlane(lo, 16)),
                 min(__builtin_amdgcn_readlane(lo, 32), __builtin_amdgcn_readlane(lo, 48)));
        hi = max(max(__builtin_amdgcn_readlane(hi, 0), __builtin_amdgcn_readlane(hi, 16)),
                 max(__builtin_amdgcn_readlane(hi, 32), __builtin_amdgcn_readlane(hi, 48)));
        if (lane == 0) {
          mn_cc_add(P, S, s_root, s_val, lp_acc, r.x, P.C, s0, 256);
          mn_cc_cls(s_min, s_max, clsmin, clsmax, r.x, s0, lo, hi);
        }
#else
        if ((lane & 15) == 0) mn_cc_add(P, S, s_root, s_val, lp_acc, r.x, P.C, s0, 64);
        const int lo = mn_row16_min(lo1), hi = -mn_row16_min(-hi1);
        if ((lane & 15) == 0) mn_cc_cls(s_min, s_max, clsmin, clsmax, r.x, s0, lo, hi);
#endif
      } else {
        mn_cc_add(P, S, s_root, s_val, lp_acc, r.x, P.C, s0, 4);
        mn_cc_cls(s_min, s_max, clsmin, clsmax, r.x, s0, lo1, hi1);
      }
    } else {
      s_q[atomicAdd(&s_qn, 1)] = i;
    }
  }
  }
  __syncthreads();
  {
    const int nq = s_qn;
    for (int t = threadIdx.x; t < nq * P.C; t += MN_CC_SUM_THREADS) {
      const int item = t / P.C, c = t - item * P.C;
      const int g = s_q[item];
      if (clean) {
        const uchar4 cl = *reinterpret_cast<const uchar4*>(clean + 4 * (size_t)g);
        const unsigned char clj[4] = {cl.x, cl.y, cl.z, cl.w};
        const uchar4 bq = *reinterpret_cast<const uchar4*>(cls0 + 4 * (size_t)g);
        const unsigned char bj[4] = {bq.x, bq.y, bq.z, bq.w};
        for (int j = 0; j < 4; j++) {
          const int px = 4 * g + j;
          if (!clj[j]) { if (c == 0) S.osize[px] = 1; continue; }
          const int rt = mn_cc_root_ro(S.parent, px);
          const int sl = mn_lds_root_slot(s_root, rt);
          const float v = mn_ld_class(P, c, px);
          mn_cc_add(P, S, s_root, s_val, lp_acc, rt, c, sl, (i64)__float2int_rn(logf(v) * (float)MN_LP_FIX));
          if (c == 0) {
            mn_cc_add(P, S, s_root, s_val, lp_acc, rt, P.C, sl, 1);
            mn_cc_cls(s_min, s_max, clsmin, clsmax, rt, sl, bj[j], bj[j]);
          }
        }
        continue;
      }
      int4 r;
      r.x = mn_cc_root_ro(S.parent, 4 * g); r.y = mn_cc_root_ro(S.parent, 4 * g + 1);
      r.z = mn_cc_root_ro(S.parent, 4 * g + 2); r.w = mn_cc_root_ro(S.parent, 4 * g + 3);
      const int s0 = mn_lds_root_slot(s_root, r.x), s1 = mn_lds_root_slot(s_root, r.y);
      const int s2 = mn_lds_root_slot(s_root, r.z), s3 = mn_lds_root_slot(s_root, r.w);
      const float4 v = mn_ld_class4(P, c, 4 * g);
      mn_cc_sums_pixelwise(P, S, s_root, s_val, lp_acc, r, c, s0, s1, s2, s3, v);
      if (c == 0) {
        const uchar4 b = *reinterpret_cast<const uchar4*>(cls0 + 4 * (size_t)g);
        mn_cc_add(P, S, s_root, s_val, lp_acc, r.x, P.C, s0, 1);
        mn_cc_add(P, S, s_root, s_val, lp_acc, r.y, P.C, s1, 1);
        mn_cc_add(P, S, s_root, s_val, lp_acc, r.z, P.C, s2, 1);
        mn_cc_add(P, S, s_root, s_val, lp_acc, r.w, P.C, s3, 1);
        mn_cc_cls(s_min, s_max, clsmin, clsmax, r.x, s0, b.x, b.x);
        mn_cc_cls(s_min, s_max, clsmin, clsmax, r.y, s1, b.y, b.y);
        mn_cc_cls(s_min, s_max, clsmin, clsmax, r.z, s2, b.z, b.z);
        mn_cc_cls(s_min, s_max, clsmin, clsmax, r.w, s3, b.w, b.w);
      }
    }
  }
  __syncthreads();
  if (threadIdx.x < MN_CC_SUM_SLOTS && s_root[threadIdx.x] >= 0) {
    atomicMin(&clsmin[s_root[threadIdx.x]], s_min[threadIdx.x]);
    atomicMax(&clsmax[s_root[threadIdx.x]], s_max[threadIdx.x]);
  }
  for (int j = threadIdx.x; j < nval; j += MN_CC_SUM_THREADS) {
    const u64 v = s_val[j];
    if (v == 0) continue;
    const int slot = j / (P.C + 1), c = j - slot * (P.C + 1);
    mn_cc_add(P, S, s_root, s_val, lp_acc, s_root[slot], c, -1, (i64)v);
  }
}

__device__ __forceinline__ bool mn_tab_insert_bounded(const HashTab& T, u64 key, i64 s,
                                                      int* __restrict__ tcount = nullptr,
                                                      int count = 0) {
  unsigned slot = mn_hash(key) & T.mask;
#pragma unroll 1
  for (int t = 0; t < 256; t++) {
    const u64 prev = atomicCAS(&T.key[slot], MN_EMPTY, key);
    if (prev == MN_EMPTY || prev == key) {
      atomicAdd(reinterpret_cast<u64*>(&T.S[slot]), (u64)s);
      if (tcount) atomicAdd(&tcount[slot], count);
      T.touched[slot] = 1;
      return true;
    }
    slot = (slot + 1) & T.mask;
  }
  return false;
}

#define MN_CC_EDGE_SLOTS 256
__device__ __forceinline__ bool mn_cc_lds_add_cnt(u64* s_key, u64* s_sum, int* s_cnt, const HashTab& T,
                                                  int* __restrict__ tcount, u64 key, i64 s, int n) {
  unsigned h = (mn_hash(key) >> 7) & (MN_CC_EDGE_SLOTS - 1);
#pragma unroll 1
  for (int t = 0; t < 32; t++) {
    u64 prev = s_key[h];
    if (prev == MN_EMPTY) prev = atomicCAS(&s_key[h], MN_EMPTY, key);
    if (prev == MN_EMPTY || prev == key) {
      atomicAdd(&s_sum[h], (u64)s);
      atomicAdd(&s_cnt[h], n);
      return true;
    }
    h = (h + 1) & (MN_CC_EDGE_SLOTS - 1);
  }
  return mn_tab_insert_bounded(T, key, s, tcount, n);
}


#define MN_CC_CROSS_THREADS 256
template <int PX>
__global__ __launch_bounds__(MN_CC_CROSS_THREADS) void mn_cc_cross(
    ImgParams P, const int* __restrict__ parent, HashTab T, const unsigned* __restrict__ negbits,
    int* __restrict__ violations, int* __restrict__ tcount) {
  constexpr int QCAP = MN_CC_CROSS_THREADS * PX * MN_MAX_OFFSETS > 10240 ? 10240 : MN_CC_CROSS_THREADS * PX * MN_MAX_OFFSETS;
  __shared__ unsigned short s_item[QCAP];
  __shared__ int s_w[MN_CC_CROSS_THREADS / 64];
  __shared__ u64 s_key[MN_CC_EDGE_SLOTS];
  __shared__ u64 s_sum[MN_CC_EDGE_SLOTS];
  __shared__ int s_cnt[MN_CC_EDGE_SLOTS];
  const int lane = threadIdx.x & 63, wave = threadIdx.x >> 6;
  const int ngroups = (P.N + PX - 1) / PX;
  const int i = blockIdx.x * MN_CC_CROSS_THREADS + threadIdx.x;
  unsigned ng[PX];
#pragma unroll
  for (int j = 0; j < PX; j++) ng[j] = 0u;
  if (i < ngroups) {
    if (PX == 4) {
      const uint4 t = *reinterpret_cast<const uint4*>(negbits + 4 * (size_t)i);
      ng[0] = t.x; ng[1 % PX] = t.y; ng[2 % PX] = t.z; ng[3 % PX] = t.w;
    } else {
      ng[0] = negbits[i];
    }
  }
  int nneg = 0;
#pragma unroll
  for (int j = 0; j < PX; j++) nneg += __popc(ng[j]);
  int incl = nneg;
#pragma unroll
  for (int off = 1; off < 64; off <<= 1) {
    const int t = __shfl_up(incl, off);
    if (lane >= off) incl += t;
  }
  if (lane == 63) s_w[wave] = incl;
  if (threadIdx.x < MN_CC_EDGE_SLOTS) {
    s_key[threadIdx.x] = MN_EMPTY; s_sum[threadIdx.x] = 0; s_cnt[threadIdx.x] = 0;
  }
  __syncthreads();
  int woff = 0, total = 0;
#pragma unroll
  for (int w = 0; w < MN_CC_CROSS_THREADS / 64; w++) { if (w < wave) woff += s_w[w]; total += s_w[w]; }
  if (total == 0) return;
  int bad = 0, over = 0;
  for (int q0 = 0; q0 < total; q0 += QCAP) {
    int pos = woff + incl - nneg - q0;
#pragma unroll
    for (int j = 0; j < PX; j++) {
      unsigned bitsleft = ng[j];
      while (bitsleft) {
        const int k = __ffs((int)bitsleft) - 1;
        bitsleft &= bitsleft - 1u;
        if (pos >= 0 && pos < QCAP) s_item[pos] = (unsigned short)(((threadIdx.x * PX + j) << 5) | k);
        pos++;
      }
    }
    __syncthreads();
    const int nq = min(QCAP, total - q0);
    for (int t0 = 0; t0 < nq; t0 += MN_CC_CROSS_THREADS) {
      const int t = t0 + threadIdx.x;
      u64 key = MN_EMPTY;
      i64 sx = 0;
      if (t < nq) {
        const unsigned it = s_item[t];
        const int k = (int)(it & 31u);
        const int p = blockIdx.x * (MN_CC_CROSS_THREADS * PX) + (int)(it >> 5);
        const int q = p + P.di[k] * P.W + P.dj[k];
        const float x = mn_same_value(P, mn_ld_same(P, k, p));
        const int ru = parent[p], rv = parent[q];
        if (ru == rv) bad++;
        else {
          key = mn_key(ru, rv);
          sx = mn_edge_fixed(x);
        }
      }
      const u64 k0 = ((u64)(unsigned)__shfl((int)(key >> 32), 0) << 32) | (u64)(unsigned)__shfl((int)(key & 0xFFFFFFFFull), 0);
      if (__ballot(key != k0) == 0) {
        if (k0 == MN_EMPTY) continue;
        i64 tot = sx;
        for (int off = 32; off > 0; off >>= 1) tot += __shfl_xor(tot, off);
        if (lane == 0 && !mn_cc_lds_add_cnt(s_key, s_sum, s_cnt, T, tcount, k0, tot, 64)) over++;
      } else if (key != MN_EMPTY) {
        if (!mn_cc_lds_add_cnt(s_key, s_sum, s_cnt, T, tcount, key, sx, 1)) over++;
      }
    }
    __syncthreads();
  }
  if (threadIdx.x < MN_CC_EDGE_SLOTS && s_key[threadIdx.x] != MN_EMPTY)
    if (!mn_tab_insert_bounded(T, s_key[threadIdx.x], (i64)s_sum[threadIdx.x], tcount, s_cnt[threadIdx.x]))
      over++;
  for (int off = 32; off > 0; off >>= 1) { bad += __shfl_xor(bad, off); over += __shfl_xor(over, off); }
  if ((threadIdx.x & 63) == 0) {
    if (bad) atomicAdd(violations, bad);
    if (over) atomicAdd(violations + 1, over);
  }
}

__device__ __forceinline__ void mn_cc_finish_root(const ImgParams& P, const ObjState& S, int p,
                                                  const i64* __restrict__ lp_acc,
                                                  const int* __restrict__ clsmin,
                                                  const int* __restrict__ clsmax,
                                                  int* __restrict__ compsize, int* __restrict__ rootlist,
                                                  int* __restrict__ nroots, int* __restrict__ violations,
                                                  const unsigned char* __restrict__ cls0) {
  if (S.parent[p] != p) return;
  if (cls0) {
    S.ocls[p] = cls0[p];
    S.lpvalid[p] = 0;
  }
  if (rootlist) {
    rootlist[atomicAdd(nroots, 1)] = p;
    compsize[p] = S.osize[p];
    if (clsmin[p] != clsmax[p]) atomicAdd(violations, 1);
  }
  if (S.osize[p] <= 1) return;
  for (int c = 0; c < P.C; c++)
    S.lpsum[(size_t)c * P.N + p] = (float)((double)lp_acc[(size_t)c * P.N + p] * (1.0 / MN_LP_FIX));
  S.lpvalid[p] = 1;
}

__global__ __launch_bounds__(256) void mn_cc_finish(ImgParams P, ObjState S,
                                                    const unsigned char* __restrict__ cand,
                                                    const i64* __restrict__ lp_acc,
                                                    const int* __restrict__ clsmin,
                                                    const int* __restrict__ clsmax,
                                                    int* __restrict__ compsize,
                                                    int* __restrict__ rootlist,
                                                    int* __restrict__ nroots,
                                                    int* __restrict__ violations,
                                                    const unsigned char* __restrict__ cls0) {
  const int i = blockIdx.x * blockDim.x + threadIdx.x;
  const int n16 = P.N >> 4;
  if (i < n16) {
    const uint4 f = *reinterpret_cast<const uint4*>(cand + 16 * (size_t)i);
    if ((f.x | f.y | f.z | f.w) != 0u) {
      const unsigned w[4] = {f.x, f.y, f.z, f.w};
      for (int j = 0; j < 16; j++)
        if ((w[j >> 2] >> (8 * (j & 3))) & 0xFFu)
          mn_cc_finish_root(P, S, 16 * i + j, lp_acc, clsmin, clsmax, compsize, rootlist, nroots, violations, cls0);
    }
  }
  if (i < P.N - (n16 << 4)) {
    const int p = (n16 << 4) + i;
    if (cand[p]) mn_cc_finish_root(P, S, p, lp_acc, clsmin, clsmax, compsize, rootlist, nroots, violations, cls0);
  }
}

#define MN_CC_CERT_THREADS 1024
__device__ __forceinline__ void mn_cc_certificate_run(
    const ImgParams& P, const ObjState& S, const unsigned char* __restrict__ cls0,
    const int* __restrict__ compsize, const int* __restrict__ rootlist, int n, int nb_edges,
    const double* __restrict__ partial_edges, const Counters* __restrict__ cnt,
    double* __restrict__ out, int* __restrict__ violations) {
  __shared__ double sh[2][MN_CC_CERT_THREADS];
  __shared__ u64 s_cls;
  __shared__ int s_bad;
  if (threadIdx.x == 0) { s_cls = 0; s_bad = 0; }
  __syncthreads();
  i64 t_cls = 0;
  int bad_cls = 0;
  for (int j = threadIdx.x; j < n; j += MN_CC_CERT_THREADS) {
    const int p = rootlist[j];
    int f = p;
    while (S.parent[f] != f) f = S.parent[f];
    const int oc = S.ocls[f];
    if (cls0[p] != oc) bad_cls += compsize[p];
    if (f == p) t_cls += __float2ll_rn(mn_obj_lp(P, S, S.lpvalid[p] != 0, p, oc) * 4294967296.0f);
  }
  if (t_cls) atomicAdd(&s_cls, (u64)t_cls);
  if (bad_cls) atomicAdd(&s_bad, bad_cls);
  double a0 = 0.0, a1 = 0.0;
  for (int b = threadIdx.x; b < nb_edges; b += MN_CC_CERT_THREADS) {
    a0 += partial_edges[(size_t)b * 2];
    a1 += partial_edges[(size_t)b * 2 + 1];
  }
  sh[0][threadIdx.x] = a0; sh[1][threadIdx.x] = a1;
  __syncthreads();
  for (int off = MN_CC_CERT_THREADS / 2; off > 0; off >>= 1) {
    if (threadIdx.x < off) { sh[0][threadIdx.x] += sh[0][threadIdx.x + off]; sh[1][threadIdx.x] += sh[1][threadIdx.x + off]; }
    __syncthreads();
  }
  if (threadIdx.x == 0) {
    const double cls_term = (double)(i64)s_cls * (1.0 / 4294967296.0);
    const double moved = (double)cnt->merged_S * (1.0 / MN_FIX_ONE);
    out[0] = cls_term + ((sh[1][0] + sh[0][0]) + moved) * (double)P.omf;
    out[1] = cls_term; out[2] = sh[0][0]; out[3] = sh[1][0];
    if (cnt->merged_E) atomicAdd(violations, cnt->merged_E);
    if (s_bad) atomicAdd(violations + 3, s_bad);
  }
  __syncthreads();
}

__global__ __launch_bounds__(MN_CC_CERT_THREADS) void mn_cc_certificate(
    ImgParams P, ObjState S, const unsigned char* __restrict__ cls0, const int* __restrict__ compsize,
    const int* __restrict__ rootlist, const int* __restrict__ nroots, int nb_edges,
    const double* __restrict__ partial_edges, const Counters* __restrict__ cnt,
    double* __restrict__ out, int* __restrict__ violations) {
  mn_cc_certificate_run(P, S, cls0, compsize, rootlist, *nroots, nb_edges, partial_edges, cnt, out, violations);
}
```

mergenet_amd/labels.py:

```python

from __future__ import annotations

import numpy as np


def canonical(labels: np.ndarray) -> np.ndarray:
    flat = np.asarray(labels).reshape(-1)
    _, first, inv = np.unique(flat, return_index=True, return_inverse=True)
    order = np.argsort(np.argsort(first))
    return order[inv].reshape(np.asarray(labels).shape).astype(np.int64)


def same_partition(a: np.ndarray, b: np.ndarray) -> bool:
    return bool(np.array_equal(canonical(a), canonical(b)))


def partition_mismatch(a: np.ndarray, b: np.ndarray) -> int:
    ca, cb = canonical(a).reshape(-1), canonical(b).reshape(-1)
    pairs, counts = np.unique(np.stack([ca, cb], 1), axis=0, return_counts=True)
    best_a = {}
    for (x, y), n in zip(pairs, counts):
        if n > best_a.get(x, (None, 0))[1]:
            best_a[x] = (y, n)
    used = {}
    good = 0
    for x, (y, n) in best_a.items():
        if y in used:
            continue
        size_a = int((ca == x).sum())
        size_b = int((cb == y).sum())
        if size_a == n and size_b == n:
            good += n
            used[y] = x
    return int(ca.size - good)


def masks_equivalent(mask_a, classes_a, mask_b, classes_b) -> bool:
    ma, mb = np.asarray(mask_a), np.asarray(mask_b)
    if ma.shape != mb.shape or len(classes_a) != len(classes_b):
        return False
    if not np.array_equal(ma == 0, mb == 0):
        return False
    if not same_partition(ma, mb):
        return False
    flat_a, flat_b = ma.reshape(-1), mb.reshape(-1)
    _, idx = np.unique(flat_a, return_index=True)
    for i in idx:
        la, lb = int(flat_a[i]), int(flat_b[i])
        if la == 0:
            continue
        if classes_a[la - 1] != classes_b[lb - 1]:
            return False
    return True


def agreement(mask_a, mask_b) -> int:
    a = np.asarray(mask_a).astype(np.int64).reshape(-1)
    b = np.asarray(mask_b).astype(np.int64).reshape(-1)
    cont = np.zeros((int(a.max()) + 1, int(b.max()) + 1), np.int64)
    np.add.at(cont, (a, b), 1)
    agree = 0
    for _ in range(min(cont.shape)):
        i, j = np.unravel_index(int(np.argmax(cont)), cont.shape)
        if cont[i, j] <= 0:
            break
        agree += int(cont[i, j])
        cont[i, :] = -1
        cont[:, j] = -1
    return agree



def instance_table(mask: np.ndarray, num_instances: int) -> np.ndarray:
    m = np.asarray(mask)
    H, W = m.shape
    table = np.empty((int(num_instances), 5), np.int32)
    for k in range(1, int(num_instances) + 1):
        ys, xs = np.nonzero(m == k)
        if ys.size == 0:
            table[k - 1] = (0, W, H, -1, -1)
        else:
            table[k - 1] = (ys.size, xs.min(), ys.min(), xs.max(), ys.max())
    return table


def filter_instances(mask: np.ndarray, class_table, num_instances: int, table: np.ndarray, min_area: int,
                     scores=None, min_score=None):
    m = np.asarray(mask)
    K = int(num_instances)
    table = np.asarray(table)
    classes = np.asarray(class_table)
    remap = np.zeros(K + 1, np.int32)
    kept = []
    for k in range(1, K + 1):
        keep = table[k - 1][0] >= min_area
        if scores is not None:
            keep = keep and bool(scores[k - 1] >= (-np.inf if min_score is None else min_score))
        if keep:
            kept.append(k)
            remap[k] = len(kept)
    out = np.zeros(m.shape, np.int32)
    for k in kept:
        out[m == k] = remap[k]
    new_classes = np.full(K, -1, np.int32)
    new_table = np.empty((len(kept), 5), np.int32)
    for k in kept:
        new_classes[remap[k] - 1] = classes[k - 1]
        new_table[remap[k] - 1] = table[k - 1]
    new_scores = None
    if scores is not None:
        new_scores = np.asarray([scores[k - 1] for k in kept], np.float32)
    return out, new_classes, new_scores, new_table, len(kept), remap
```

Measured before the change: 16310.

## Add lean sweep form with per-64-pixel uniform group sums and packed bits

```diff
diff --git a/mergenet_amd/csrc/mergenet_hip.hip b/mergenet_amd/csrc/mergenet_hip.hip
--- a/mergenet_amd/csrc/mergenet_hip.hip
+++ b/mergenet_amd/csrc/mergenet_hip.hip
@@ -127,6 +127,7 @@
     hipGraphExec_t eA, eB;
     hipStream_t cap;
     Queued queued;
+    int lean_form;
   } replay;
   hipStream_t side;
   hipEvent_t ev_fork;
@@ -724,8 +725,22 @@
 #endif
 }
 
+static bool sweep_lean_form(const mn_context* c, const ImgParams& P, int px) {
+  return px >= 4 && !(c->debug_flags & 512) && P.N >= 64 && gsum_stride(P.N) == (size_t)P.N;
+}
+static LeanOut lean_out(const ImgParams& P, bool lean_form) {
+  LeanOut LO = {-1, 0, 0, 0};
+  if (!lean_form) return LO;
+  for (int k = 0; k < P.O; k++)
+    if (P.di[k] == 0 && P.dj[k] == 1) { LO.kh = k; break; }
+  LO.packed = P.O <= 16 ? 1 : 0;
+  LO.rec0 = (P.N / 4 + 1) & ~1;
+  LO.flag0 = LO.rec0 + 2 * ((P.N + 63) / 64);
+  return LO;
+}
+
 template <int PX, int DT, bool LG = false>
-static void launch_sign(mn_context* c, const ImgParams& P, hipStream_t st, bool cls, bool lean_cls) {
+static void launch_sign(mn_context* c, const ImgParams& P, hipStream_t st, bool cls, bool lean_cls, bool lean_form) {
   const int N = P.N, ngroups = (N + PX - 1) / PX;
   const dim3 g(grid_for(ngroups, MN_CC_SIGN_THREADS)), b(MN_CC_SIGN_THREADS);
   ClsOut CO;
@@ -733,19 +748,23 @@
   CO.gsum = reinterpret_cast<int*>(c->lpsum);
   CO.gstride = gsum_stride(P.N);
   const bool plain = (DT != MN_DTYPE_F32 || LG || !P.clip) && P.sdb == 0.0f;
-#define MN_LAUNCH_SIGN(PLAINV, CLSV)                                                                    \
+  lean_form = lean_form && lean_cls && cls && PX >= 4;
+  const LeanOut LO = lean_out(P, lean_form);
+#define MN_LAUNCH_SIGN(PLAINV, CLSV, LEANV)                                                             \
   do {                                                                                                \
     if (c->ext_events)                                                                                \
-      hipExtLaunchKernelGGL((mn_cc_sign<PX, PLAINV, (CLSV) && PX >= 4, DT, LG>), g, b, 0, st, c->ev[0], c->ev[10], 0, \
-                            P, c->cc_bits, c->cc_negbits, c->scalars + 6, c->partial, CO); \
+      hipExtLaunchKernelGGL((mn_cc_sign<PX, PLAINV, (CLSV) && PX >= 4, DT, LG, (LEANV) && PX >= 4>), g, b, 0, st, \
+                            c->ev[0], c->ev[10], 0, P, c->cc_bits, c->cc_negbits, c->scalars + 6, c->partial, CO, LO); \
     else                                                                                              \
-      hipLaunchKernelGGL((mn_cc_sign<PX, PLAINV, (CLSV) && PX >= 4, DT, LG>), g, b, 0, st, P, c->cc_bits, c->cc_negbits, \
-                         c->scalars + 6, c->partial, CO);                                             \
+      hipLaunchKernelGGL((mn_cc_sign<PX, PLAINV, (CLSV) && PX >= 4, DT, LG, (LEANV) && PX >= 4>), g, b, 0, st, P, \
+                         c->cc_bits, c->cc_negbits, c->scalars + 6, c->partial, CO, LO);              \
   } while (0)
-  if (plain && cls) MN_LAUNCH_SIGN(true, true);
-  else if (plain) MN_LAUNCH_SIGN(true, false);
-  else if (cls) MN_LAUNCH_SIGN(false, true);
-  else MN_LAUNCH_SIGN(false, false);
+  if (plain && lean_form) MN_LAUNCH_SIGN(true, true, true);
+  else if (lean_form) MN_LAUNCH_SIGN(false, true, true);
+  else if (plain && cls) MN_LAUNCH_SIGN(true, true, false);
+  else if (plain) MN_LAUNCH_SIGN(true, false, false);
+  else if (cls) MN_LAUNCH_SIGN(false, true, false);
+  else MN_LAUNCH_SIGN(false, false, false);
 #undef MN_LAUNCH_SIGN
 }
 
@@ -758,23 +777,25 @@
 }
 
 template <bool LG>
-static void launch_sweep_lg(mn_context* c, const ImgParams& P, hipStream_t st, int px, bool cls, bool lean_cls) {
-#define MN_SWEEP_DT(PXV)                                                                         \
-  do {                                                                                           \
-    if (P.dtype == MN_DTYPE_F16) launch_sign<PXV, MN_DTYPE_F16, LG>(c, P, st, cls, lean_cls);    \
-    else launch_sign<PXV, MN_DTYPE_BF16, LG>(c, P, st, cls, lean_cls);                           \
+static void launch_sweep_lg(mn_context* c, const ImgParams& P, hipStream_t st, int px, bool cls, bool lean_cls,
+                            bool lean_form) {
+#define MN_SWEEP_DT(PXV)                                                                                   \
+  do {                                                                                                     \
+    if (P.dtype == MN_DTYPE_F16) launch_sign<PXV, MN_DTYPE_F16, LG>(c, P, st, cls, lean_cls, lean_form);   \
+    else launch_sign<PXV, MN_DTYPE_BF16, LG>(c, P, st, cls, lean_cls, lean_form);                          \
   } while (0)
   if (P.dtype == MN_DTYPE_F32) {
-    if (px == 4) launch_sign<4, MN_DTYPE_F32, LG>(c, P, st, cls, lean_cls);
-    else launch_sign<1, MN_DTYPE_F32, LG>(c, P, st, false, false);
+    if (px == 4) launch_sign<4, MN_DTYPE_F32, LG>(c, P, st, cls, lean_cls, lean_form);
+    else launch_sign<1, MN_DTYPE_F32, LG>(c, P, st, false, false, false);
   } else if (px == 8) MN_SWEEP_DT(8);
   else if (px == 4) MN_SWEEP_DT(4);
-  else { cls = false; lean_cls = false; MN_SWEEP_DT(1); }
+  else { cls = false; lean_cls = false; lean_form = false; MN_SWEEP_DT(1); }
 #undef MN_SWEEP_DT
 }
-static void launch_sweep(mn_context* c, const ImgParams& P, hipStream_t st, int px, bool cls, bool lean_cls) {
-  if (P.logits) launch_sweep_lg<true>(c, P, st, px, cls, lean_cls);
-  else launch_sweep_lg<false>(c, P, st, px, cls, lean_cls);
+static void launch_sweep(mn_context* c, const ImgParams& P, hipStream_t st, int px, bool cls, bool lean_cls,
+                         bool lean_form = false) {
+  if (P.logits) launch_sweep_lg<true>(c, P, st, px, cls, lean_cls, lean_form);
+  else launch_sweep_lg<false>(c, P, st, px, cls, lean_cls, lean_form);
 }
 
 template <int PX>
@@ -821,7 +842,10 @@
   int* clsmax = c->mapbuf;
   const bool fused_cls = sweep4;
   const bool lean_cls = fused_cls && !cores;
-  launch_sweep(c, P, st, px, fused_cls, lean_cls);
+  const bool lean_form = lean_cls && sweep_lean_form(c, P, px);
+  const LeanOut LO = lean_out(P, lean_form);
+  if (c->replay.capturing) c->replay.lean_form = lean_form ? 1 : 0;
+  launch_sweep(c, P, st, px, fused_cls, lean_cls, lean_form);
   if (!few_events && !c->ext_events) MN_HIP(hipEventRecord(c->ev[10], st));
   const unsigned* lbits = c->cc_bits;
   unsigned kshort = 0u;
@@ -886,10 +910,16 @@
                                  hipFuncAttributeMaxDynamicSharedMemorySize, (int)lds));
       MN_HIP(hipFuncSetAttribute(reinterpret_cast<const void*>(mn_cc_sums),
                                  hipFuncAttributeMaxDynamicSharedMemorySize, (int)lds));
+      MN_HIP(hipFuncSetAttribute(reinterpret_cast<const void*>(mn_cc_sums_lean),
+                                 hipFuncAttributeMaxDynamicSharedMemorySize, (int)lds));
       c->cc_sum_lds = lds;
     }
     const unsigned blocks = grid_for((size_t)(N >> 2) > 0 ? (size_t)(N >> 2) : 1, MN_CC_SUM_THREADS);
-    if (fused_cls)
+    if (lean_form)
+      hipLaunchKernelGGL(mn_cc_sums_lean, dim3((unsigned)grid_for((size_t)(N + 63) / 64, MN_CC_LEAN_GROUPS)),
+                         dim3(MN_CC_LEAN_THREADS), lds, st, P, S, (const unsigned char*)c->cls0,
+                         (const int*)reinterpret_cast<int*>(c->lpsum), gsum_stride(P.N), LO, c->lp_acc, clsmin, clsmax);
+    else if (fused_cls)
       hipLaunchKernelGGL(mn_cc_sums, dim3((blocks + MN_CC_SUMS_ITERS - 1) / MN_CC_SUMS_ITERS), dim3(MN_CC_SUM_THREADS), lds, st, P, S,
                          (const unsigned char*)c->cls0, (const int*)reinterpret_cast<int*>(c->lpsum), gsum_stride(P.N),
                          c->lp_acc, clsmin, clsmax, cores ? (const unsigned char*)c->pruned : (const unsigned char*)nullptr);
@@ -900,12 +930,14 @@
   if (!few_events && !lean) MN_HIP(hipEventRecord(c->ev[8], st));
   if (!cores)
   {
+    const bool packed = lean_form && LO.packed;
+    const unsigned* negsrc = packed ? (const unsigned*)c->cc_bits : (const unsigned*)c->cc_negbits;
     if (sweep4)
       hipLaunchKernelGGL(mn_cc_cross<4>, dim3((unsigned)grid_for((size_t)N / 4, MN_CC_CROSS_THREADS)), dim3(MN_CC_CROSS_THREADS),
-                         0, st, P, (const int*)c->parent, T, (const unsigned*)c->cc_negbits, c->scalars + 6, c->cc_tcount);
+                         0, st, P, (const int*)c->parent, T, negsrc, packed ? 16 : 0, lean_form && !MN_CC_LEAN_FLAT ? 1 : 0, c->scalars + 6, c->cc_tcount);
     else
       hipLaunchKernelGGL(mn_cc_cross<1>, dim3((unsigned)grid_for((size_t)N, MN_CC_CROSS_THREADS)), dim3(MN_CC_CROSS_THREADS),
-                         0, st, P, (const int*)c->parent, T, (const unsigned*)c->cc_negbits, c->scalars + 6, c->cc_tcount);
+                         0, st, P, (const int*)c->parent, T, negsrc, 0, 0, c->scalars + 6, c->cc_tcount);
   }
   if (!few_events && !lean) MN_HIP(hipEventRecord(c->ev[9], st));
   hipLaunchKernelGGL(mn_cc_finish, dim3(grid_for((size_t)(N >> 4) > 0 ? (size_t)(N >> 4) : 1, 256)), b, 0, st, P, S,
@@ -1773,7 +1805,7 @@
   c->cores_used = 0;
   const bool timed = !(call.opts.debug_flags & 2) && !c->ext_events;
   if (timed) MN_HIP(hipEventRecord(c->ev[0], st));
-  launch_sweep(c, P, st, sweep_px(c, P), true, true);
+  launch_sweep(c, P, st, sweep_px(c, P), true, true, c->replay.lean_form != 0);
   if (timed) MN_HIP(hipEventRecord(c->ev[10], st));
   MN_HIP(hipGraphLaunch(c->replay.eA, st));
   MN_HIP(hipEventRecord(c->ev_fork, st));
@@ -2138,7 +2170,8 @@
     for (int i = 0; i < n; i++) {
       call.d_class = d_class_pred[i % n_inputs]; call.d_adj = d_adj_pred[i % n_inputs];
       fill_params(&P, call);
-      launch_sweep(c, P, st, sweep_px(c, P), true, true);
+      const int px = sweep_px(c, P);
+      launch_sweep(c, P, st, px, true, true, sweep_lean_form(c, P, px));
     }
     if (phase == 1) MN_HIP(hipEventRecord(c->ev[1], st));
   }
diff --git a/mergenet_amd/csrc/mn_kernels_cc.h b/mergenet_amd/csrc/mn_kernels_cc.h
--- a/mergenet_amd/csrc/mn_kernels_cc.h
+++ b/mergenet_amd/csrc/mn_kernels_cc.h
@@ -103,6 +103,32 @@
   unsigned char* ocls; unsigned char* cls0; unsigned char* lpvalid; int* gsum; size_t gstride;
 };
 
+struct LeanOut { int kh; int packed; int rec0; int flag0; };
+#ifndef MN_CC_LEAN_FLAT
+#define MN_CC_LEAN_FLAT 1
+#endif
+
+template <int GL>
+__device__ __forceinline__ int mn_group_sum32(int x) {
+  x += __builtin_amdgcn_update_dpp(0, x, 0xB1, 0xF, 0xF, false);
+  x += __builtin_amdgcn_update_dpp(0, x, 0x4E, 0xF, 0xF, false);
+  x += __builtin_amdgcn_update_dpp(0, x, 0x141, 0xF, 0xF, false);
+  if constexpr (GL == 16) x += __builtin_amdgcn_update_dpp(0, x, 0x140, 0xF, 0xF, false);
+  return x;
+}
+template <int GL>
+__device__ __forceinline__ int mn_group_min(int x) {
+  x = min(x, __builtin_amdgcn_update_dpp(x, x, 0xB1, 0xF, 0xF, false));
+  x = min(x, __builtin_amdgcn_update_dpp(x, x, 0x4E, 0xF, 0xF, false));
+  x = min(x, __builtin_amdgcn_update_dpp(x, x, 0x141, 0xF, 0xF, false));
+  if constexpr (GL == 16) x = min(x, __builtin_amdgcn_update_dpp(x, x, 0x140, 0xF, 0xF, false));
+  return x;
+}
+template <int GL>
+__device__ __forceinline__ i64 mn_group_sum_exact(int lo, int hi) {
+  return ((i64)mn_group_sum32<GL>(hi) << 16) + (i64)mn_group_sum32<GL>(lo);
+}
+
 __device__ __forceinline__ int mn_cc_argmax_logf(const ImgParams& P, int p) {
   float best = 0.0f;
   int b = 0;
@@ -126,8 +152,9 @@
   return b;
 }
 
-template <int DT, bool LG = false>
-__device__ __forceinline__ void mn_cc_class_part(const ImgParams& P, const ClsOut& CO, int i) {
+template <int DT, bool LG = false, bool LEAN = false>
+__device__ __forceinline__ void mn_cc_class_part(const ImgParams& P, const ClsOut& CO, int i, bool uni = false,
+                                                 const LeanOut& LO = LeanOut()) {
   float4 best, prev = make_float4(-1.0f, -1.0f, -1.0f, -1.0f);
   int b0 = 0, b1 = 0, b2 = 0, b3 = 0;
   float4 nxt = mn_ld_stream4_t<DT, LG>(P.cls, 4 * (size_t)i);
@@ -144,6 +171,16 @@
       if (v.z > best.z) { prev.z = best.z; best.z = v.z; b2 = c; }
       if (v.w > best.w) { prev.w = best.w; best.w = v.w; b3 = c; }
     }
+    if constexpr (LEAN) {
+      const int gv = __float2int_rn(logf((v.x * v.y) * (v.z * v.w)) * 16777216.0f);
+      if (uni) {
+        const i64 gs = mn_group_sum_exact<16>(gv & 0xFFFF, gv >> 16);
+        if ((threadIdx.x & 15) == 0)
+          *reinterpret_cast<i64*>(&CO.gsum[(size_t)c * CO.gstride + LO.rec0 + 2 * (size_t)(i >> 4)]) = gs;
+      } else {
+        mn_st_stream(&CO.gsum[(size_t)c * CO.gstride + i], gv);
+      }
+    } else
     mn_st_stream(&CO.gsum[(size_t)c * CO.gstride + i], __float2int_rn(logf((v.x * v.y) * (v.z * v.w)) * 16777216.0f));
   }
   const float near = 1.0f - 3.814697265625e-06f;
@@ -156,10 +193,20 @@
   if (CO.ocls) *reinterpret_cast<uchar4*>(CO.ocls + 4 * (size_t)i) = o;
   *reinterpret_cast<uchar4*>(CO.cls0 + 4 * (size_t)i) = o;
   if (CO.lpvalid) *reinterpret_cast<uchar4*>(CO.lpvalid + 4 * (size_t)i) = make_uchar4(0, 0, 0, 0);
-}
-
-template <int DT, bool LG = false>
-__device__ __forceinline__ void mn_cc_class_part8(const ImgParams& P, const ClsOut& CO, int i) {
+  if constexpr (LEAN) {
+    int word = 0;
+    if (uni) {
+      const int lo = mn_group_min<16>(min(min(b0, b1), min(b2, b3)));
+      const int hi = -mn_group_min<16>(-max(max(b0, b1), max(b2, b3)));
+      word = 1 | (lo << 8) | (hi << 16);
+    }
+    if ((threadIdx.x & 15) == 0) CO.gsum[LO.flag0 + (i >> 4)] = word;
+  }
+}
+
+template <int DT, bool LG = false, bool LEAN = false>
+__device__ __forceinline__ void mn_cc_class_part8(const ImgParams& P, const ClsOut& CO, int i, bool uni = false,
+                                                  const LeanOut& LO = LeanOut()) {
   float best[8], prev[8];
   int b[8];
 #pragma unroll
@@ -179,6 +226,15 @@
     int2 g;
     g.x = __float2int_rn(logf((v[0] * v[1]) * (v[2] * v[3])) * 16777216.0f);
     g.y = __float2int_rn(logf((v[4] * v[5]) * (v[6] * v[7])) * 16777216.0f);
+    if constexpr (LEAN) {
+      if (uni) {
+        const i64 gs = mn_group_sum_exact<8>((g.x & 0xFFFF) + (g.y & 0xFFFF), (g.x >> 16) + (g.y >> 16));
+        if ((threadIdx.x & 7) == 0)
+          *reinterpret_cast<i64*>(&CO.gsum[(size_t)c * CO.gstride + LO.rec0 + 2 * (size_t)(i >> 3)]) = gs;
+      } else {
+        *reinterpret_cast<int2*>(&CO.gsum[(size_t)c * CO.gstride + 2 * (size_t)i]) = g;
+      }
+    } else
     *reinterpret_cast<int2*>(&CO.gsum[(size_t)c * CO.gstride + 2 * (size_t)i]) = g;
   }
   const float near = 1.0f - 3.814697265625e-06f;
@@ -191,19 +247,31 @@
   if (CO.ocls) *reinterpret_cast<uint2*>(CO.ocls + 8 * (size_t)i) = o;
   *reinterpret_cast<uint2*>(CO.cls0 + 8 * (size_t)i) = o;
   if (CO.lpvalid) *reinterpret_cast<uint2*>(CO.lpvalid + 8 * (size_t)i) = make_uint2(0u, 0u);
-}
-
-template <int PX, bool PLAIN, bool CLS, int DT = MN_DTYPE_F32, bool LG = false>
+  if constexpr (LEAN) {
+    int word = 0;
+    if (uni) {
+      int lo1 = b[0], hi1 = b[0];
+#pragma unroll
+      for (int j = 1; j < 8; j++) { lo1 = min(lo1, b[j]); hi1 = max(hi1, b[j]); }
+      const int lo = mn_group_min<8>(lo1), hi = -mn_group_min<8>(-hi1);
+      word = 1 | (lo << 8) | (hi << 16);
+    }
+    if ((threadIdx.x & 7) == 0) CO.gsum[LO.flag0 + (i >> 3)] = word;
+  }
+}
+
+template <int PX, bool PLAIN, bool CLS, int DT = MN_DTYPE_F32, bool LG = false, bool LEAN = false>
 __global__ __launch_bounds__(MN_CC_SIGN_THREADS) void mn_cc_sign(
     ImgParams P, unsigned* __restrict__ bits, unsigned* __restrict__ negbits, int* __restrict__ violations,
-    double* __restrict__ partial, ClsOut CO) {
+    double* __restrict__ partial, ClsOut CO, LeanOut LO) {
+  static_assert(!LEAN || (CLS && PX >= 4), "the lean form belongs to the sweep that takes the class planes");
   const int lane = threadIdx.x & 63, wave = threadIdx.x >> 6;
   const int ngroups = (P.N + PX - 1) / PX;
   const int i = blockIdx.x * MN_CC_SIGN_THREADS + threadIdx.x;
   const bool live = i < ngroups;
   const int p0 = live ? PX * i : 0;
   const int r = p0 / P.W, c0 = p0 - r * P.W;
-  if constexpr (CLS) {
+  if constexpr (CLS && !LEAN) {
     if (live) {
       if constexpr (PX == 8) mn_cc_class_part8<DT, LG>(P, CO, i);
       else mn_cc_class_part<DT, LG>(P, CO, i);
@@ -294,6 +362,15 @@
     ng[j] &= in;
     bad += __popc(in & ~(m[j] | ng[j]));
   }
+  if (LEAN && LO.packed) {
+#pragma unroll
+    for (int j = 0; j < PX; j++) m[j] |= ng[j] << 16;
+    if (live) {
+      mn_st_stream(reinterpret_cast<uint4*>(bits + p0), make_uint4(m[0], m[1 % PX], m[2 % PX], m[3 % PX]));
+      if (PX == 8)
+        mn_st_stream(reinterpret_cast<uint4*>(bits + p0) + 1, make_uint4(m[4 % PX], m[5 % PX], m[6 % PX], m[7 % PX]));
+    }
+  } else
   if (live) {
     if (PX == 8) {
       mn_st_stream(reinterpret_cast<uint4*>(bits + p0), make_uint4(m[0], m[1 % PX], m[2 % PX], m[3 % PX]));
@@ -306,6 +383,20 @@
     } else {
       bits[p0] = m[0];
       negbits[p0] = ng[0];
+    }
+  }
+  if constexpr (LEAN) {
+    constexpr int GL = 64 / PX;
+    const unsigned hb = LO.kh >= 0 ? 1u << LO.kh : 0u;
+    unsigned all = live ? hb : 0u;
+#pragma unroll
+    for (int j = 0; j < PX - 1; j++) all &= m[j];
+    if ((lane & (GL - 1)) != GL - 1) all &= m[PX - 1];
+    const unsigned long long bal = __ballot(all != 0u);
+    const bool uni = ((unsigned)(bal >> (lane & ~(GL - 1))) & ((1u << GL) - 1u)) == ((1u << GL) - 1u);
+    if (live) {
+      if constexpr (PX == 8) mn_cc_class_part8<DT, LG, true>(P, CO, i, uni, LO);
+      else mn_cc_class_part<DT, LG, true>(P, CO, i, uni, LO);
     }
   }
   for (int off = 32; off > 0; off >>= 1) {
@@ -851,6 +942,48 @@
   mn_cc_add(P, S, s_root, s_val, lp_acc, r.w, c, s3, (i64)__float2int_rn(logf(vw) * (float)MN_LP_FIX));
 }
 
+__device__ __forceinline__ void mn_cc_sums_boundary_item(const ImgParams& P, const ObjState& S, int* s_root,
+                                                         u64* s_val, int* s_min, int* s_max,
+                                                         const unsigned char* __restrict__ cls0,
+                                                         i64* __restrict__ lp_acc, int* __restrict__ clsmin,
+                                                         int* __restrict__ clsmax, int g, int c) {
+  int4 r;
+  r.x = mn_cc_root_ro(S.parent, 4 * g); r.y = mn_cc_root_ro(S.parent, 4 * g + 1);
+  r.z = mn_cc_root_ro(S.parent, 4 * g + 2); r.w = mn_cc_root_ro(S.parent, 4 * g + 3);
+  const int s0 = mn_lds_root_slot(s_root, r.x), s1 = mn_lds_root_slot(s_root, r.y);
+  const int s2 = mn_lds_root_slot(s_root, r.z), s3 = mn_lds_root_slot(s_root, r.w);
+  const float4 v = mn_ld_class4(P, c, 4 * g);
+  mn_cc_sums_pixelwise(P, S, s_root, s_val, lp_acc, r, c, s0, s1, s2, s3, v);
+  if (c == 0) {
+    const uchar4 b = *reinterpret_cast<const uchar4*>(cls0 + 4 * (size_t)g);
+    mn_cc_add(P, S, s_root, s_val, lp_acc, r.x, P.C, s0, 1);
+    mn_cc_add(P, S, s_root, s_val, lp_acc, r.y, P.C, s1, 1);
+    mn_cc_add(P, S, s_root, s_val, lp_acc, r.z, P.C, s2, 1);
+    mn_cc_add(P, S, s_root, s_val, lp_acc, r.w, P.C, s3, 1);
+    mn_cc_cls(s_min, s_max, clsmin, clsmax, r.x, s0, b.x, b.x);
+    mn_cc_cls(s_min, s_max, clsmin, clsmax, r.y, s1, b.y, b.y);
+    mn_cc_cls(s_min, s_max, clsmin, clsmax, r.z, s2, b.z, b.z);
+    mn_cc_cls(s_min, s_max, clsmin, clsmax, r.w, s3, b.w, b.w);
+  }
+}
+
+template <int THREADS>
+__device__ __forceinline__ void mn_cc_sums_flush(const ImgParams& P, const ObjState& S, int* s_root, u64* s_val,
+                                                 int* s_min, int* s_max, i64* __restrict__ lp_acc,
+                                                 int* __restrict__ clsmin, int* __restrict__ clsmax) {
+  const int nval = MN_CC_SUM_SLOTS * (P.C + 1);
+  if (threadIdx.x < MN_CC_SUM_SLOTS && s_root[threadIdx.x] >= 0) {
+    atomicMin(&clsmin[s_root[threadIdx.x]], s_min[threadIdx.x]);
+    atomicMax(&clsmax[s_root[threadIdx.x]], s_max[threadIdx.x]);
+  }
+  for (int j = threadIdx.x; j < nval; j += THREADS) {
+    const u64 v = s_val[j];
+    if (v == 0) continue;
+    const int slot = j / (P.C + 1), c = j - slot * (P.C + 1);
+    mn_cc_add(P, S, s_root, s_val, lp_acc, s_root[slot], c, -1, (i64)v);
+  }
+}
+
 __global__ __launch_bounds__(MN_CC_SUM_THREADS) void mn_cc_sums(
     ImgParams P, ObjState S, const unsigned char* __restrict__ cls0, const int* __restrict__ gsum,
     size_t gstride, i64* __restrict__ lp_acc, int* __restrict__ clsmin, int* __restrict__ clsmax,
@@ -962,37 +1095,113 @@
         }
         continue;
       }
-      int4 r;
-      r.x = mn_cc_root_ro(S.parent, 4 * g); r.y = mn_cc_root_ro(S.parent, 4 * g + 1);
-      r.z = mn_cc_root_ro(S.parent, 4 * g + 2); r.w = mn_cc_root_ro(S.parent, 4 * g + 3);
-      const int s0 = mn_lds_root_slot(s_root, r.x), s1 = mn_lds_root_slot(s_root, r.y);
-      const int s2 = mn_lds_root_slot(s_root, r.z), s3 = mn_lds_root_slot(s_root, r.w);
-      const float4 v = mn_ld_class4(P, c, 4 * g);
-      mn_cc_sums_pixelwise(P, S, s_root, s_val, lp_acc, r, c, s0, s1, s2, s3, v);
-      if (c == 0) {
-        const uchar4 b = *reinterpret_cast<const uchar4*>(cls0 + 4 * (size_t)g);
-        mn_cc_add(P, S, s_root, s_val, lp_acc, r.x, P.C, s0, 1);
-        mn_cc_add(P, S, s_root, s_val, lp_acc, r.y, P.C, s1, 1);
-        mn_cc_add(P, S, s_root, s_val, lp_acc, r.z, P.C, s2, 1);
-        mn_cc_add(P, S, s_root, s_val, lp_acc, r.w, P.C, s3, 1);
-        mn_cc_cls(s_min, s_max, clsmin, clsmax, r.x, s0, b.x, b.x);
-        mn_cc_cls(s_min, s_max, clsmin, clsmax, r.y, s1, b.y, b.y);
-        mn_cc_cls(s_min, s_max, clsmin, clsmax, r.z, s2, b.z, b.z);
-        mn_cc_cls(s_min, s_max, clsmin, clsmax, r.w, s3, b.w, b.w);
-      }
-    }
-  }
-  __syncthreads();
-  if (threadIdx.x < MN_CC_SUM_SLOTS && s_root[threadIdx.x] >= 0) {
-    atomicMin(&clsmin[s_root[threadIdx.x]], s_min[threadIdx.x]);
-    atomicMax(&clsmax[s_root[threadIdx.x]], s_max[threadIdx.x]);
-  }
-  for (int j = threadIdx.x; j < nval; j += MN_CC_SUM_THREADS) {
-    const u64 v = s_val[j];
-    if (v == 0) continue;
-    const int slot = j / (P.C + 1), c = j - slot * (P.C + 1);
-    mn_cc_add(P, S, s_root, s_val, lp_acc, s_root[slot], c, -1, (i64)v);
-  }
+      mn_cc_sums_boundary_item(P, S, s_root, s_val, s_min, s_max, cls0, lp_acc, clsmin, clsmax, g, c);
+    }
+  }
+  __syncthreads();
+  mn_cc_sums_flush<MN_CC_SUM_THREADS>(P, S, s_root, s_val, s_min, s_max, lp_acc, clsmin, clsmax);
+}
+
+#define MN_CC_LEAN_THREADS 256
+#define MN_CC_LEAN_GROUPS 64
+__global__ __launch_bounds__(MN_CC_LEAN_THREADS) void mn_cc_sums_lean(
+    ImgParams P, ObjState S, const unsigned char* __restrict__ cls0, const int* __restrict__ gsum,
+    size_t gstride, LeanOut LO, i64* __restrict__ lp_acc, int* __restrict__ clsmin, int* __restrict__ clsmax) {
+  extern __shared__ __attribute__((aligned(16))) unsigned char cc_smem[];
+  u64* s_val = reinterpret_cast<u64*>(cc_smem);
+  __shared__ int s_root[MN_CC_SUM_SLOTS];
+  __shared__ int s_min[MN_CC_SUM_SLOTS];
+  __shared__ int s_max[MN_CC_SUM_SLOTS];
+  __shared__ int s_grp[MN_CC_LEAN_GROUPS];
+  __shared__ int s_q[MN_CC_LEAN_GROUPS * 16];
+  __shared__ int s_ngrp, s_qn;
+  const int nval = MN_CC_SUM_SLOTS * (P.C + 1);
+  for (int i = threadIdx.x; i < nval; i += MN_CC_LEAN_THREADS) s_val[i] = 0;
+  if (threadIdx.x == 0) { s_ngrp = 0; s_qn = 0; }
+  if (threadIdx.x < MN_CC_SUM_SLOTS) { s_root[threadIdx.x] = -1; s_min[threadIdx.x] = 255; s_max[threadIdx.x] = 0; }
+  __syncthreads();
+  constexpr int G = MN_CC_SUMS_G;
+  const int n4 = P.N >> 2, ngroups = (n4 + 15) >> 4;
+  const int g0 = blockIdx.x * MN_CC_LEAN_GROUPS;
+  if (threadIdx.x < MN_CC_LEAN_GROUPS && g0 + (int)threadIdx.x < ngroups) {
+    const int grp = g0 + (int)threadIdx.x;
+    const int word = gsum[LO.flag0 + grp];
+    if (word & 1) {
+      const int root = mn_cc_root_ro(S.parent, 64 * grp);
+      const int s0 = mn_lds_root_slot(s_root, root);
+      for (int c0 = 0; c0 < P.C; c0 += G) {
+        i64 v[G];
+#pragma unroll
+        for (int a = 0; a < G; a++)
+          v[a] = c0 + a < P.C ? *reinterpret_cast<const i64*>(&gsum[(size_t)(c0 + a) * gstride + LO.rec0 + 2 * (size_t)grp]) : 0;
+#pragma unroll
+        for (int a = 0; a < G; a++) {
+          if (c0 + a >= P.C) break;
+          mn_cc_add(P, S, s_root, s_val, lp_acc, root, c0 + a, s0, v[a]);
+        }
+      }
+      mn_cc_add(P, S, s_root, s_val, lp_acc, root, P.C, s0, 64);
+      mn_cc_cls(s_min, s_max, clsmin, clsmax, root, s0, (word >> 8) & 255, (word >> 16) & 255);
+    } else {
+      s_grp[atomicAdd(&s_ngrp, 1)] = (int)threadIdx.x;
+    }
+  }
+  __syncthreads();
+  const int nlanes = s_ngrp * 16;
+  for (int t = threadIdx.x; t < nlanes; t += MN_CC_LEAN_THREADS) {
+    const int i = (g0 + s_grp[t >> 4]) * 16 + (t & 15);
+    if (i >= n4) continue;
+    int4 r = *reinterpret_cast<const int4*>(S.parent + 4 * (size_t)i);
+    const uchar4 b = *reinterpret_cast<const uchar4*>(cls0 + 4 * (size_t)i);
+    int g[G];
+#pragma unroll
+    for (int a = 0; a < G; a++) g[a] = a < P.C ? gsum[(size_t)a * gstride + i] : 0;
+    r.x = mn_cc_root_ro(S.parent, r.x);
+    r.y = r.y == r.x ? r.x : mn_cc_root_ro(S.parent, r.y);
+    r.z = r.z == r.x ? r.x : mn_cc_root_ro(S.parent, r.z);
+    r.w = r.w == r.x ? r.x : mn_cc_root_ro(S.parent, r.w);
+    if (r.x == r.y && r.x == r.z && r.x == r.w) {
+      const int s0 = mn_lds_root_slot(s_root, r.x);
+      for (int c0 = 0; c0 < P.C; c0 += G) {
+        if (c0 > 0) {
+#pragma unroll
+          for (int a = 0; a < G; a++) g[a] = c0 + a < P.C ? gsum[(size_t)(c0 + a) * gstride + i] : 0;
+        }
+#pragma unroll
+        for (int a = 0; a < G; a++) {
+          if (c0 + a >= P.C) break;
+          mn_cc_add(P, S, s_root, s_val, lp_acc, r.x, c0 + a, s0, (i64)g[a]);
+        }
+      }
+      mn_cc_add(P, S, s_root, s_val, lp_acc, r.x, P.C, s0, 4);
+      mn_cc_cls(s_min, s_max, clsmin, clsmax, r.x, s0, min(min((int)b.x, (int)b.y), min((int)b.z, (int)b.w)),
+                max(max((int)b.x, (int)b.y), max((int)b.z, (int)b.w)));
+    } else {
+      s_q[atomicAdd(&s_qn, 1)] = i;
+    }
+  }
+#if MN_CC_LEAN_FLAT
+  for (int t = threadIdx.x; t < MN_CC_LEAN_GROUPS * 16; t += MN_CC_LEAN_THREADS) {
+    const int i = g0 * 16 + t;
+    if (i >= n4) continue;
+    int4 r = *reinterpret_cast<const int4*>(S.parent + 4 * (size_t)i);
+    const int4 r_in = r;
+    r.x = mn_cc_root_ro(S.parent, r.x);
+    r.y = r.y == r_in.x ? r.x : mn_cc_root_ro(S.parent, r.y);
+    r.z = r.z == r_in.x ? r.x : mn_cc_root_ro(S.parent, r.z);
+    r.w = r.w == r_in.x ? r.x : mn_cc_root_ro(S.parent, r.w);
+    if (r.x != r_in.x || r.y != r_in.y || r.z != r_in.z || r.w != r_in.w)
+      *reinterpret_cast<int4*>(S.parent + 4 * (size_t)i) = r;
+  }
+#endif
+  __syncthreads();
+  const int nq = s_qn;
+  for (int t = threadIdx.x; t < nq * P.C; t += MN_CC_LEAN_THREADS) {
+    const int item = t / P.C;
+    mn_cc_sums_boundary_item(P, S, s_root, s_val, s_min, s_max, cls0, lp_acc, clsmin, clsmax, s_q[item], t - item * P.C);
+  }
+  __syncthreads();
+  mn_cc_sums_flush<MN_CC_LEAN_THREADS>(P, S, s_root, s_val, s_min, s_max, lp_acc, clsmin, clsmax);
 }
 
 __device__ __forceinline__ bool mn_tab_insert_bounded(const HashTab& T, u64 key, i64 s,
@@ -1035,8 +1244,8 @@
 #define MN_CC_CROSS_THREADS 256
 template <int PX>
 __global__ __launch_bounds__(MN_CC_CROSS_THREADS) void mn_cc_cross(
-    ImgParams P, const int* __restrict__ parent, HashTab T, const unsigned* __restrict__ negbits,
-    int* __restrict__ violations, int* __restrict__ tcount) {
+    ImgParams P, const int* __restrict__ parent, HashTab T, const unsigned* __restrict__ negbits, int shift,
+    int chase, int* __restrict__ violations, int* __restrict__ tcount) {
   constexpr int QCAP = MN_CC_CROSS_THREADS * PX * MN_MAX_OFFSETS > 10240 ? 10240 : MN_CC_CROSS_THREADS * PX * MN_MAX_OFFSETS;
   __shared__ unsigned short s_item[QCAP];
   __shared__ int s_w[MN_CC_CROSS_THREADS / 64];
@@ -1052,9 +1261,9 @@
   if (i < ngroups) {
     if (PX == 4) {
       const uint4 t = *reinterpret_cast<const uint4*>(negbits + 4 * (size_t)i);
-      ng[0] = t.x; ng[1 % PX] = t.y; ng[2 % PX] = t.z; ng[3 % PX] = t.w;
+      ng[0] = t.x >> shift; ng[1 % PX] = t.y >> shift; ng[2 % PX] = t.z >> shift; ng[3 % PX] = t.w >> shift;
     } else {
-      ng[0] = negbits[i];
+      ng[0] = negbits[i] >> shift;
     }
   }
   int nneg = 0;
@@ -1100,7 +1309,7 @@
         const int p = blockIdx.x * (MN_CC_CROSS_THREADS * PX) + (int)(it >> 5);
         const int q = p + P.di[k] * P.W + P.dj[k];
         const float x = mn_same_value(P, mn_ld_same(P, k, p));
-        const int ru = parent[p], rv = parent[q];
+        const int ru = chase ? mn_cc_root_ro(parent, p) : parent[p], rv = chase ? mn_cc_root_ro(parent, q) : parent[q];
         if (ru == rv) bad++;
         else {
           key = mn_key(ru, rv);
diff --git a/mergenet_amd/labels.py b/mergenet_amd/labels.py
--- a/mergenet_amd/labels.py
+++ b/mergenet_amd/labels.py
@@ -111,3 +111,19 @@
     if scores is not None:
         new_scores = np.asarray([scores[k - 1] for k in kept], np.float32)
     return out, new_classes, new_scores, new_table, len(kept), remap
+
+
+
+def uniform_groups(pos_bits: np.ndarray, offsets) -> np.ndarray:
+    bits = np.asarray(pos_bits).astype(np.int64).reshape(-1) & 0xFFFFFFFF
+    n = bits.size
+    groups = (n + 63) // 64
+    flags = np.zeros(groups, bool)
+    offs = [(int(i), int(j)) for (i, j) in offsets]
+    if (0, 1) not in offs:
+        return flags
+    k = offs.index((0, 1))
+    link = ((bits >> k) & 1).astype(bool)
+    full = n // 64
+    flags[:full] = link[: full * 64].reshape(full, 64)[:, :63].all(axis=1)
+    return flags
```

Result: faster. 16780 (median of 6 runs) (+2.9%).
